# preshanth/rfi_toolbox

Measured on AMD Instinct MI355X. Metric: training patches/sec (128x128x3), higher is better.
Workload: dtype f32; 1 GPU; UNet(3,1,32) train step (fwd+BCE/dice+bwd+clip+Adam), batch 64/GPU x 128x128x3 NHWC, BASELINE configs[1] shape on the reference's U-Net (the '3-layer CNN' of configs[1] is not in the reference; its builder-defined form runs with --workload cnn3); global_batch=64, parallelism=dp1, params=7765985

## Files before the change

rfi_toolbox_amd/csrc/api.cpp:

```cpp
#include <dlfcn.h>

#include <algorithm>
#include <cmath>

#include "model.hpp"

using namespace rfi;

namespace rfi {
static thread_local std::string g_last_error;
void set_last_error(const std::string& msg) { g_last_error = msg; }
}

void rfi_ctx::activate() const { RFI_CHECK_HIP(hipSetDevice(device)); }

void* rfi_ctx::alloc(size_t bytes) {
    void* p = nullptr;
    if (bytes == 0) bytes = 16;
    RFI_CHECK_HIP(hipMalloc(&p, bytes));
    allocs[p] = bytes;
    return p;
}
void rfi_ctx::release(void* p) {
    if (!p) return;
// ... 432 lines not shown
int rfi_model_set_head_sigmoid(rfi_model* m, int enabled) {
    return guarded([&] {
        RFI_REQUIRE(plain_unet(m), "set_head_sigmoid: U-Net models only");
        m->head_sigmoid = enabled != 0;
    });
}

namespace {

void copy_on_stream(rfi_ctx* ctx, void* dst, const void* src, size_t bytes, hipMemcpyKind kind) {
    if (kind == hipMemcpyDeviceToDevice) launch_copy_d2d(ctx, dst, src, bytes);
    else RFI_CHECK_HIP(hipMemcpyAsync(dst, src, bytes, kind, ctx->stream));
}
const float* stage_input(rfi_model* m, const float* x, int x_mem, int n, int h, int w, bool nchw) {
    const size_t cnt = (size_t)n * h * w * m->in_ch;
    const float* dev = x;
    if (x_mem == RFI_HOST) {
        float* st = m->buf(nchw ? m->x_stage2 : m->x_stage);
        RFI_CHECK_HIP(hipMemcpyAsync(st, x, cnt * sizeof(float), hipMemcpyHostToDevice, m->ctx->stream));
        dev = st;
    }
    if (nchw) {
        launch_nchw_to_nhwc(m->ctx, dev, n, m->in_ch, h, w, m->buf(m->x_stage));
        dev = m->buf(m->x_stage);
    }
    return dev;
}
const uint8_t* stage_labels(rfi_model* m, const uint8_t* y, int y_mem, int n, int h, int w) {
    if (y_mem == RFI_DEVICE) return y;
    uint8_t* st = reinterpret_cast<uint8_t*>(m->buf(m->lab_stage));
    RFI_CHECK_HIP(hipMemcpyAsync(st, y, (size_t)n * h * w * m->out_scale * m->out_scale, hipMemcpyHostToDevice, m->ctx->stream));
    return st;
}
void sync_if_host(rfi_model* m, int mem_a, int mem_b = RFI_DEVICE) {
    static const bool always = getenv("RFI_SYNC_ALWAYS") != nullptr;
    if (always || mem_a != RFI_DEVICE || mem_b != RFI_DEVICE) RFI_CHECK_HIP(hipStreamSynchronize(m->ctx->stream));
}
void emit_logits(rfi_model* m, float* out, int out_mem, int n, int h, int w, bool nchw) {
    h *= m->out_scale; w *= m->out_scale;
    const size_t cnt = (size_t)n * h * w * m->out_ch;
    const float* src = m->buf(m->head_sigmoid ? m->probs : m->logits);
    if (nchw && m->out_ch > 1) {
        launch_nhwc_to_nchw(m->ctx, src, n, m->out_ch, h, w, m->buf(m->out_stage));
        src = m->buf(m->out_stage);
    }
    copy_on_stream(m->ctx, out, src, cnt * sizeof(float), out_mem == RFI_DEVICE ? hipMemcpyDeviceToDevice : hipMemcpyDeviceToHost);
    sync_if_host(m, out_mem);
}
float read_scalar(rfi_model* m, const float* dev) {
    RFI_CHECK_HIP(hipMemcpyAsync(m->ctx->pinned, dev, sizeof(float), hipMemcpyDeviceToHost, m->ctx->stream));
    RFI_CHECK_HIP(hipStreamSynchronize(m->ctx->stream));
    return m->ctx->pinned[0];
}
void check_hyper(const rfi_hyper* hp) {
    RFI_REQUIRE(hp, "null hyper-parameters");
    RFI_REQUIRE(hp->lr >= 0 && hp->eps >= 0 && hp->weight_decay >= 0, "Adam: lr, eps, weight_decay must be >= 0");
    RFI_REQUIRE(hp->beta1 >= 0 && hp->beta1 < 1 && hp->beta2 >= 0 && hp->beta2 < 1, "Adam: betas must be in [0,1)");
}


void backward_with_exchange(rfi_model* m, const float* x, const uint8_t* y, int n, int h, int w) {
    struct Flag { rfi_model* m; ~Flag() { m->exchange_in_backward = false; } } flag{m};
    m->exchange_in_backward = true;
    m->backward(x, y, n, h, w);
}
void exchange_and_apply(rfi_model* m, const rfi_hyper& hp) {
    if (m->ctx->exchange_active()) {
        m->exchange_join();
        m->apply(hp, 1.0f / (float)m->ctx->exchange_world());
    } else {
        m->apply(hp, 1.0f);
    }
}

}

int rfi_model_forward_nhwc(rfi_model* m, const float* x, int x_mem, int n, int h, int w, float* logits,
                           int logits_mem) {
    return guarded([&] {
        m->ctx->activate();
        m->prepare(n, h, w);
        const float* xd = stage_input(m, x, x_mem, n, h, w, false);
        m->forward(xd, n, h, w, m->training);
        emit_logits(m, logits, logits_mem, n, h, w, false);
    });
}
int rfi_model_forward_nchw(rfi_model* m, const float* x, int x_mem, int n, int h, int w, float* logits,
                           int logits_mem) {
    return guarded([&] {
        m->ctx->activate();
        m->prepare(n, h, w);
        const float* xd = stage_input(m, x, x_mem, n, h, w, true);
        m->forward(xd, n, h, w, m->training);
        emit_logits(m, logits, logits_mem, n, h, w, true);
    });
}

int rfi_train_forward_backward(rfi_model* m, const float* x, int x_mem, const uint8_t* labels,
                               int labels_mem, int n, int h, int w, float* loss_out) {
    return guarded([&] {
        m->ctx->activate();
        m->prepare(n, h, w);
        const float* xd = stage_input(m, x, x_mem, n, h, w, false);
        const uint8_t* yd = stage_labels(m, labels, labels_mem, n, h, w);
        m->forward(xd, n, h, w, true);
        m->loss_forward(yd, n, h, w);
        m->backward(xd, yd, n, h, w);
        if (loss_out) *loss_out = m->last_loss = read_scalar(m, m->d_scalars);
    });
}
int rfi_train_apply(rfi_model* m, const rfi_hyper* hp, float grad_scale, float* grad_norm_out) {
    return guarded([&] {
        check_hyper(hp);
        m->ctx->activate();
        RFI_REQUIRE(m->pN > 0, "rfi_train_apply: no gradients (call rfi_train_forward_backward first)");
        m->apply(*hp, grad_scale);
        if (grad_norm_out) *grad_norm_out = m->last_norm = read_scalar(m, m->d_scalars + 1);
    });
}
int rfi_train_step(rfi_model* m, const float* x, int x_mem, const uint8_t* labels, int labels_mem,
                   int n, int h, int w, const rfi_hyper* hp, float* loss_out) {
    return guarded([&] {
        check_hyper(hp);
        m->ctx->activate();
        m->prepare(n, h, w);
        const float* xd = stage_input(m, x, x_mem, n, h, w, false);
        const uint8_t* yd = stage_labels(m, labels, labels_mem, n, h, w);
        m->forward(xd, n, h, w, true);
        m->loss_forward(yd, n, h, w);
        backward_with_exchange(m, xd, yd, n, h, w);
        exchange_and_apply(m, *hp);
        RFI_CHECK_HIP(hipMemcpyAsync(m->ctx->pinned, m->d_scalars, 2 * sizeof(float), hipMemcpyDeviceToHost,
                                     m->ctx->stream));
        RFI_CHECK_HIP(hipStreamSynchronize(m->ctx->stream));
        m->last_loss = m->ctx->pinned[0];
        m->last_norm = m->ctx->pinned[1];
        if (loss_out) *loss_out = m->last_loss;
    });
}
int rfi_train_step_async(rfi_model* m, const float* x_dev, const uint8_t* labels_dev, int n, int h,
                         int w, const rfi_hyper* hp) {
    return guarded([&] {
        check_hyper(hp);
        m->ctx->activate();
        m->prepare(n, h, w);
        m->forward(x_dev, n, h, w, true);
        m->loss_forward(labels_dev, n, h, w);
        backward_with_exchange(m, x_dev, labels_dev, n, h, w);
        exchange_and_apply(m, *hp);
    });
}
int rfi_model_backward_dlogits(rfi_model* m, const float* x, int x_mem, const float* dlogits, int dlogits_mem, int n, int h,
                               int w) {
    return guarded([&] {
        RFI_REQUIRE(m->gx >= 0, "backward_dlogits: mask / RPN / box heads only");
        RFI_REQUIRE(m->pN == n && m->pH == h && m->pW == w, "backward_dlogits: run the forward pass on this input first");
        m->ctx->activate();
        const float* xd = stage_input(m, x, x_mem, n, h, w, false);
        const size_t cnt = (size_t)n * h * w * m->out_scale * m->out_scale * m->out_ch;
        copy_on_stream(m->ctx, m->buf(m->dlogits), dlogits, cnt * sizeof(float),
                       dlogits_mem == RFI_DEVICE ? hipMemcpyDeviceToDevice : hipMemcpyHostToDevice);
        struct Flag { rfi_model* m; ~Flag() { m->ext_dlogits = false; } } flag{m};
        m->ext_dlogits = true;
        m->backward(xd, nullptr, n, h, w);
        sync_if_host(m, x_mem, dlogits_mem);
    });
}
int rfi_backbone_forward(rfi_model* m, const float* x, int x_mem, int n, int h, int w, float* const feats[5], int feats_mem) {
    return guarded([&] {
        auto* b = dynamic_cast<BackboneModel*>(m);
        RFI_REQUIRE(b && feats, "backbone_forward: ResNet-50-FPN models only");
        m->ctx->activate();
        m->prepare(n, h, w);
        const float* xd = stage_input(m, x, x_mem, n, h, w, false);
        m->forward(xd, n, h, w, false);
        for (int i = 0; i < 5; ++i) {
            if (!feats[i]) continue;
            const int lvl = i + 2;
            const size_t cnt = (size_t)n * (h >> lvl) * (w >> lvl) * m->out_ch;
            copy_on_stream(m->ctx, feats[i], m->buf(i < 4 ? b->fP[i] : b->fP6), cnt * sizeof(float),
                           feats_mem == RFI_DEVICE ? hipMemcpyDeviceToDevice : hipMemcpyDeviceToHost);
        }
        sync_if_host(m, x_mem, feats_mem);
    });
}
int rfi_backbone_backward(rfi_model* m, const float* x, int x_mem, int n, int h, int w, const float* const dfeats[5], int dfeats_mem) {
    return guarded([&] {
        auto* b = dynamic_cast<BackboneModel*>(m);
        RFI_REQUIRE(b && dfeats, "backbone_backward: ResNet-50-FPN models only");
        RFI_REQUIRE(m->pN == n && m->pH == h && m->pW == w, "backbone_backward: run the forward pass on this input first");
        m->ctx->activate();
        const float* xd = stage_input(m, x, x_mem, n, h, w, false);
        for (int i = 0; i < 5; ++i) {
            const int lvl = i + 2;
            const size_t cnt = (size_t)n * (h >> lvl) * (w >> lvl) * m->out_ch;
            float* dst = m->buf(i < 4 ? b->fdP[i] : b->fdP6);
            if (dfeats[i])
                copy_on_stream(m->ctx, dst, dfeats[i], cnt * sizeof(float),
// ... 757 lines not shown
```

rfi_toolbox_amd/csrc/conv_stem.hip:

```cpp
#include <algorithm>

#include "ws_common.hpp"

namespace rfi {
namespace {

using namespace ws;

struct StemDev {
    const float* x;
    int N, H, W;
    const float* w;
    const float* bias;
    float* y;
    int y_ps, Cout;
    double* stats;
};

constexpr int TH = 8, TW = 32, HH = TH + 2, HW = TW + 2, HP = HH * HW;
constexpr int PLANE = HP * 8;

template <int NT>
__global__ __launch_bounds__(256) void conv_stem_kernel(StemDev d) {
    __shared__ __attribute__((aligned(16))) unsigned char s_img[3 * PLANE];
    __shared__ double s_stat[4 * NT * 64 * 2];
    const int tid = threadIdx.x, lane = tid & 63, wave = tid >> 6;
    const int li = lane & 31, kh = lane >> 5;

    bf16x8 bfr[NT][3][3];
#pragma unroll
    for (int nt = 0; nt < NT; ++nt)
#pragma unroll
        for (int s = 0; s < 3; ++s) {
            f32x4 v[2];
#pragma unroll
            for (int h = 0; h < 2; ++h) {
                const int tap = 4 * s + 2 * kh + h, co = nt * 32 + li;
                v[h] = f32x4{0.f, 0.f, 0.f, 0.f};
                if (tap < 9 && co < d.Cout) v[h] = *reinterpret_cast<const f32x4*>(d.w + ((size_t)tap * d.Cout + co) * 4);
            }
            unsigned pl[3][4];
            split_pair(v[0].x, v[0].y, pl[0][0], pl[1][0], pl[2][0]);
            split_pair(v[0].z, v[0].w, pl[0][1], pl[1][1], pl[2][1]);
            split_pair(v[1].x, v[1].y, pl[0][2], pl[1][2], pl[2][2]);
            split_pair(v[1].z, v[1].w, pl[0][3], pl[1][3], pl[2][3]);
#pragma unroll
            for (int p = 0; p < 3; ++p) bfr[nt][s][p] = __builtin_bit_cast(bf16x8, u32x4{pl[p][0], pl[p][1], pl[p][2], pl[p][3]});
        }
    int toff[3][2];
#pragma unroll
    for (int s = 0; s < 3; ++s)
#pragma unroll
        for (int h = 0; h < 2; ++h) {
            const int tap = std::min(4 * s + 2 * kh + h, 8);
            toff[s][h] = ((tap / 3) * HW + tap % 3 + li) * 8;
        }
    float bias[NT];
#pragma unroll
    for (int nt = 0; nt < NT; ++nt) bias[nt] = (d.bias && nt * 32 + li < d.Cout) ? d.bias[nt * 32 + li] : 0.0f;
    double d1[NT], d2[NT];
#pragma unroll
    for (int nt = 0; nt < NT; ++nt) d1[nt] = d2[nt] = 0.0;

    const int tiles_x = (d.W + TW - 1) / TW, tiles_y = (d.H + TH - 1) / TH;
    const int ntiles = d.N * tiles_y * tiles_x;
    for (int t = blockIdx.x; t < ntiles; t += gridDim.x) {
        const int ox0 = (t % tiles_x) * TW, oy0 = ((t / tiles_x) % tiles_y) * TH, n = t / (tiles_x * tiles_y);
        __syncthreads();
        for (int idx = tid; idx < HP; idx += 256) {
            const int iy = oy0 - 1 + idx / HW, ix = ox0 - 1 + idx % HW;
            f32x4 v = {0.f, 0.f, 0.f, 0.f};
            if ((unsigned)iy < (unsigned)d.H && (unsigned)ix < (unsigned)d.W)
                v = *reinterpret_cast<const f32x4*>(d.x + ((size_t)(n * d.H + iy) * d.W + ix) * 4);
            unsigned h0, m0, l0, h1, m1, l1;
            split_pair(v.x, v.y, h0, m0, l0);
            split_pair(v.z, v.w, h1, m1, l1);
            *reinterpret_cast<u32x2*>(s_img + idx * 8) = u32x2{h0, h1};
            *reinterpret_cast<u32x2*>(s_img + PLANE + idx * 8) = u32x2{m0, m1};
            *reinterpret_cast<u32x2*>(s_img + 2 * PLANE + idx * 8) = u32x2{l0, l1};
        }
        __syncthreads();
#pragma unroll
        for (int rb = 0; rb < 2; ++rb) {
            const int row = 2 * wave + rb;
            const unsigned char* base = s_img + row * HW * 8;
            f32x16 acc[NT];
#pragma unroll
            for (int nt = 0; nt < NT; ++nt)
#pragma unroll
                for (int r = 0; r < 16; ++r) acc[nt][r] = 0.0f;
#pragma unroll
            for (int s = 0; s < 3; ++s) {
                bf16x8 af[3];
#pragma unroll
                for (int p = 0; p < 3; ++p) {
                    const u32x2 a0 = *reinterpret_cast<const u32x2*>(base + p * PLANE + toff[s][0]);
                    const u32x2 a1 = *reinterpret_cast<const u32x2*>(base + p * PLANE + toff[s][1]);
                    af[p] = __builtin_bit_cast(bf16x8, u32x4{a0.x, a0.y, a1.x, a1.y});
                }
#pragma unroll
                for (int nt = 0; nt < NT; ++nt) acc[nt] = mma3(af, bfr[nt][s], acc[nt]);
            }
            const int oy = oy0 + row;
#pragma unroll
            for (int nt = 0; nt < NT; ++nt) {
                const int co = nt * 32 + li;
                float s1 = 0.0f, s2 = 0.0f;
#pragma unroll
                for (int r = 0; r < 16; ++r) {
                    const int ox = ox0 + (r & 3) + 8 * (r >> 2) + 4 * kh;
                    const float v = acc[nt][r] + bias[nt];
                    if (oy < d.H && ox < d.W && co < d.Cout) {
                        d.y[((size_t)(n * d.H + oy) * d.W + ox) * d.y_ps + co] = v;
                        s1 += v;
                        s2 += v * v;
                    }
                }
                d1[nt] += (double)s1;
                d2[nt] += (double)s2;
            }
        }
    }
    if (d.stats) {
#pragma unroll
        for (int nt = 0; nt < NT; ++nt) {
            s_stat[((wave * NT + nt) * 64 + lane) * 2] = d1[nt];
            s_stat[((wave * NT + nt) * 64 + lane) * 2 + 1] = d2[nt];
        }
        __syncthreads();
        if (tid < 32 * NT && tid < d.Cout) {
            const int nt = tid >> 5, cl = tid & 31;
            double t1 = 0.0, t2 = 0.0;
#pragma unroll
            for (int w = 0; w < 4; ++w)
#pragma unroll
                for (int h = 0; h < 2; ++h) {
                    t1 += s_stat[((w * NT + nt) * 64 + h * 32 + cl) * 2];
                    t2 += s_stat[((w * NT + nt) * 64 + h * 32 + cl) * 2 + 1];
                }
            d.stats[((size_t)blockIdx.x * d.Cout + tid) * 2] = t1;
            d.stats[((size_t)blockIdx.x * d.Cout + tid) * 2 + 1] = t2;
        }
    }
}

}

bool conv_stem_eligible(const ConvArgs& a) {
    if (!(a.R == 3 && a.S == 1 && a.pad == 1 && a.zgroups == 1 && a.Cin == 4 && a.x.pstride == 4 && (a.Cout == 32 || a.Cout == 64))) return false;
    if (a.Hin != a.H || a.Win != a.W || a.Hout != a.H || a.Wout != a.W || a.osy != 1 || a.osx != 1 || a.ooy || a.oox) return false;
    if (a.xf.scale || a.fold || a.y16) return false;
    if ((reinterpret_cast<uintptr_t>(a.x.p) | reinterpret_cast<uintptr_t>(a.w)) & 15) return false;
    return (int64_t)a.N * a.H * a.W * std::max<int64_t>(a.y.pstride, 4) * 4 < ((int64_t)1 << 40);
}

void launch_conv_stem(rfi_ctx* ctx, ConvArgs& a) {
    RFI_REQUIRE(conv_stem_eligible(a) && a.bf16x3, "conv_stem: shape or arithmetic not eligible");
    const int ntiles = a.N * (int)cdiv(a.H, TH) * (int)cdiv(a.W, TW);
    int GX = std::min(ntiles, 1024);
    if (a.stats && GX > a.stats_max_records) GX = a.stats_max_records > 0 ? a.stats_max_records : GX;
    if (a.stats && a.stats_max_records > 0) a.stats_records = GX;
    else { a.stats = nullptr; a.stats_records = 0; }
    StemDev d{a.x.p, a.N, a.H, a.W, a.w, a.bias, a.y.p, (int)a.y.pstride, a.Cout, a.stats};
    const double flops = a.algo_flops >= 0 ? a.algo_flops : 2.0 * a.N * a.H * a.W * 9.0 * 3 * a.Cout;
    const double bytes = 4.0 * ((double)a.N * a.H * a.W * (4 + a.Cout) + 9.0 * 4 * a.Cout);
    std::string label;
    if (ctx->profiling)
        label = "conv_stem N" + std::to_string(a.N) + " " + std::to_string(a.H) + "x" + std::to_string(a.W) + " 4->" + std::to_string(a.Cout) +
                " 3xbf16";
    ProfScope ps(ctx, FAM_CONV_MFMA, flops, bytes, label);
    if (a.Cout == 32) hipLaunchKernelGGL(conv_stem_kernel<1>, dim3(GX), dim3(256), 0, ctx->stream, d);
    else hipLaunchKernelGGL(conv_stem_kernel<2>, dim3(GX), dim3(256), 0, ctx->stream, d);
    check_launch("conv_stem");
}

}
```

rfi_toolbox_amd/csrc/elem_kernels.hip:

```cpp
#include <hip/hip_ext.h>

#include "kernels.hpp"

namespace rfi {

namespace {

constexpr int kBlock = 256;
constexpr int kFinCh = 2;
constexpr int kFinLanes = kBlock / kFinCh;

__device__ __forceinline__ double wave_sum(double v) {
#pragma unroll
    for (int o = 32; o > 0; o >>= 1) v += __shfl_down(v, o, 64);
    return v;
}

__device__ __forceinline__ double finish_sum(double v, double* red) {
#pragma unroll
    for (int o = 32; o >= kFinCh; o >>= 1) v += __shfl_xor(v, o, 64);
    const int wave = threadIdx.x >> 6, lane = threadIdx.x & 63;
    __syncthreads();
    if (lane < kFinCh) red[wave * kFinCh + lane] = v;
    __syncthreads();
// ... 71 lines not shown
        v[e] = (float)h;
    }
    *reinterpret_cast<uint2*>(p) = make_uint2((unsigned)q[0] | ((unsigned)q[1] << 16), (unsigned)q[2] | ((unsigned)q[3] << 16));
}
template <int V, int NQ>
__device__ __forceinline__ void row_lane_reduce(double (&acc)[NQ][V], double* red, int CL, int RL, int cl,
                                                int rl) {
#pragma unroll
    for (int q = 0; q < NQ; ++q)
#pragma unroll
        for (int v = 0; v < V; ++v) red[(q * V + v) * kBlock + threadIdx.x] = acc[q][v];
    __syncthreads();
    const int NF = RL >= 4 ? 4 : 1;
    if (rl < NF) {
#pragma unroll
        for (int q = 0; q < NQ; ++q)
#pragma unroll
            for (int v = 0; v < V; ++v) {
                double t0 = rl == 0 ? acc[q][v] : 0.0, t1 = 0.0;
                const double* rp = red + (q * V + v) * kBlock + cl;
                int k = rl == 0 ? NF : rl;
                for (; k + NF < RL; k += 2 * NF) {
                    t0 += rp[k * CL];
                    t1 += rp[(k + NF) * CL];
                }
                if (k < RL) t0 += rp[k * CL];
                acc[q][v] = t0 + t1;
            }
    }
    if (NF > 1) {
        __syncthreads();
        if (rl > 0 && rl < NF) {
#pragma unroll
            for (int q = 0; q < NQ; ++q)
#pragma unroll
                for (int v = 0; v < V; ++v) red[(q * V + v) * kBlock + threadIdx.x] = acc[q][v];
        }
        __syncthreads();
        if (rl == 0) {
#pragma unroll
            for (int q = 0; q < NQ; ++q)
#pragma unroll
                for (int v = 0; v < V; ++v) {
                    double t = acc[q][v];
                    for (int j = 1; j < NF; ++j) t += red[(q * V + v) * kBlock + j * CL + cl];
                    acc[q][v] = t;
                }
        }
    }
}

__device__ __forceinline__ float act_f(float a, float slope) { return a > 0.0f ? a : (slope != 0.0f ? a * slope : 0.0f); }
__device__ __forceinline__ float dact_f(float z, float g, float slope) { return z > 0.0f ? g : g * slope; }

template <int V>
__global__ void bn_stats_kernel(const float* __restrict__ y, int64_t M, int C, int CL,
                                int64_t rows_per_block, double* __restrict__ partial) {
    __shared__ double red[2 * V * kBlock];
    const int RL = kBlock / CL;
    const int cl = threadIdx.x % CL, rl = threadIdx.x / CL;
    const int c = (blockIdx.y * CL + cl) * V;
    const int64_t r0 = (int64_t)blockIdx.x * rows_per_block;
    int64_t r1 = r0 + rows_per_block;
    if (r1 > M) r1 = M;
    double acc[2][V];
#pragma unroll
    for (int v = 0; v < V; ++v) acc[0][v] = acc[1][v] = 0;
    if (c < C) {
        for (int64_t r = r0 + rl; r < r1; r += RL) {
            float x[V];
            ldv<V>(y + r * C + c, x);
#pragma unroll
            for (int v = 0; v < V; ++v) {
                const double d = (double)x[v];
                acc[0][v] += d;
                acc[1][v] += d * d;
            }
        }
    }
    row_lane_reduce<V, 2>(acc, red, CL, RL, cl, rl);
    if (rl == 0 && c < C) {
#pragma unroll
        for (int v = 0; v < V; ++v) {
            partial[((int64_t)blockIdx.x * C + c + v) * 2 + 0] = acc[0][v];
            partial[((int64_t)blockIdx.x * C + c + v) * 2 + 1] = acc[1][v];
        }
    }
}

__global__ void bn_finalize_kernel(const double* __restrict__ partial, int records, int C,
                                   double count, const float* __restrict__ gamma,
                                   const float* __restrict__ beta, float* __restrict__ running_mean,
                                   float* __restrict__ running_var, int ema_repeats,
                                   float* __restrict__ mean_out, float* __restrict__ invstd_out,
                                   float* __restrict__ scale, float* __restrict__ shift,
                                   float* __restrict__ var_out) {
    __shared__ double red[2 * kBlock];
    const int cl = threadIdx.x & (kFinCh - 1), rl = threadIdx.x / kFinCh;
    const int c = blockIdx.x * kFinCh + cl;
    double s1 = 0, s2 = 0;
    if (c < C) {
        for (int r = rl; r < records; r += kFinLanes) {
            s1 += partial[((int64_t)r * C + c) * 2 + 0];
            s2 += partial[((int64_t)r * C + c) * 2 + 1];
        }
    }
// ... 197 lines not shown
                        o[v] = g[v] * (dz - k1[v] - xh * k2[v]);
                        if (SUMS) p1[v] += o[v];
                    }
                    *reinterpret_cast<uint4*>(planes + r * pl_stride + c) =
                        make_uint4(pack_bf16x2(o[0], o[1]), pack_bf16x2(o[2], o[3]), pack_bf16x2(o[4], o[5]), pack_bf16x2(o[6], o[7]));
                }
            }
            if (SUMS) {
#pragma unroll
                for (int v = 0; v < 8; ++v) acc[0][v] += (double)p1[v];
            }
        }
    }
    if constexpr (SUMS) {
        row_lane_reduce<8, 1>(acc, red, CL, RL, cl, rl);
        if (rl == 0 && c < C) {
#pragma unroll
            for (int v = 0; v < 8; ++v) partial[(int64_t)blockIdx.x * C + c + v] = acc[0][v];
        }
    }
}

__global__ void bn_bwd_finalize_kernel(const double* __restrict__ partial, int records, int C,
                                       double count, float* c1, float* c2, float* dgamma,
                                       float* dbeta) {
    __shared__ double red[2 * kBlock];
    const int cl = threadIdx.x & (kFinCh - 1), rl = threadIdx.x / kFinCh;
    const int c = blockIdx.x * kFinCh + cl;
    double s1 = 0, s2 = 0;
    if (c < C) {
        for (int r = rl; r < records; r += kFinLanes) {
            s1 += partial[((int64_t)r * C + c) * 2 + 0];
            s2 += partial[((int64_t)r * C + c) * 2 + 1];
        }
    }
    s1 = finish_sum(s1, red);
    s2 = finish_sum(s2, red);
    if (rl == 0 && c < C) {
        c1[c] = (float)(s1 / count);
        c2[c] = (float)(s2 / count);
        dgamma[c] = (float)s2;
        dbeta[c] = (float)s1;
    }
}

template <int V>
__global__ void bn_bwd_apply_kernel(void* __restrict__ da_, int da16, const void* __restrict__ y, int y16, int64_t yps, int64_t M,
                                    int C, int CL, int64_t rows_per_block,
                                    const float* __restrict__ scale, const float* __restrict__ shift,
                                    const float* __restrict__ mean, const float* __restrict__ invstd,
                                    const float* __restrict__ gamma, const float* __restrict__ c1,
                                    const float* __restrict__ c2, double* __restrict__ partial, float slope,
                                    unsigned short* __restrict__ planes, int64_t pl_stride, int P,
                                    const float* __restrict__ head_dl, const float* __restrict__ head_w) {
    __shared__ double red[V * kBlock];
    const int RL = kBlock / CL;
    const int cl = threadIdx.x % CL, rl = threadIdx.x / CL;
    const int c = (blockIdx.y * CL + cl) * V;
    const int64_t r0 = (int64_t)blockIdx.x * rows_per_block;
    int64_t r1 = r0 + rows_per_block;
    if (r1 > M) r1 = M;
    double acc[1][V];
#pragma unroll
    for (int v = 0; v < V; ++v) acc[0][v] = 0;
    if (c < C) {
        float sc[V], sh[V], mu[V], is[V], g[V], k1[V], k2[V];
        ldv<V>(scale + c, sc); ldv<V>(shift + c, sh); ldv<V>(mean + c, mu); ldv<V>(invstd + c, is);
        ldv<V>(gamma + c, g); ldv<V>(c1 + c, k1); ldv<V>(c2 + c, k2);
#pragma unroll
        for (int v = 0; v < V; ++v) g[v] = g[v] * is[v];
        float hw[V];
#pragma unroll
        for (int v = 0; v < V; ++v) hw[v] = head_dl ? head_w[c + v] : 0.0f;
        constexpr int U = 4;
        for (int64_t rb = r0 + rl; rb < r1; rb += (int64_t)U * RL) {
          float yu[U][V], du[U][V];
#pragma unroll
          for (int k = 0; k < U; ++k) {
              const int64_t r = rb + (int64_t)k * RL;
              if (r < r1) {
                  ldy<V>(y, y16, r * yps + c, yu[k]);
                  if (head_dl) {
                      const float d = head_dl[r];
#pragma unroll
                      for (int v = 0; v < V; ++v) du[k][v] = d * hw[v];
                  } else {
                      ldy<V>(da_, da16, r * C + c, du[k]);
                  }
              }
          }
#pragma unroll
          for (int k = 0; k < U; ++k) {
            const int64_t r = rb + (int64_t)k * RL;
            if (r >= r1) break;
            float yv[V], dv[V], o[V];
#pragma unroll
            for (int v = 0; v < V; ++v) { yv[v] = yu[k][v]; dv[v] = du[k][v]; }
#pragma unroll
            for (int v = 0; v < V; ++v) {
                const float dz = dact_f(yv[v] * sc[v] + sh[v], dv[v], slope);
                const float xh = (yv[v] - mu[v]) * is[v];
                o[v] = g[v] * (dz - k1[v] - xh * k2[v]);
                acc[0][v] += (double)o[v];
            }
            if (planes) {
                unsigned short* q = planes + r * pl_stride + (int64_t)(c >> 4) * (P * 16) + (c & 15);
                float res[V];
#pragma unroll
                for (int v = 0; v < V; ++v) res[v] = o[v];
                for (int p = 0; p < P; ++p) {
                    unsigned short hq[V];
#pragma unroll
                    for (int v = 0; v < V; ++v) {
                        const __bf16 h = (__bf16)res[v];
                        hq[v] = __builtin_bit_cast(unsigned short, h);
                        res[v] -= (float)h;
                    }
                    if constexpr (V == 4)
                        *reinterpret_cast<uint2*>(q + p * 16) = make_uint2((unsigned)hq[0] | ((unsigned)hq[1] << 16), (unsigned)hq[2] | ((unsigned)hq[3] << 16));
                    else
                        q[p * 16] = hq[0];
                }
            } else {
                stv<V>(static_cast<float*>(da_) + r * C + c, o);
            }
          }
        }
    }
    row_lane_reduce<V, 1>(acc, red, CL, RL, cl, rl);
    if (rl == 0 && c < C) {
#pragma unroll
        for (int v = 0; v < V; ++v) partial[(int64_t)blockIdx.x * C + c + v] = acc[0][v];
    }
}

__global__ void finish_channel_sum_kernel(const double* __restrict__ partial, int records,
// ... 236 lines not shown
         i += (int64_t)gridDim.x * blockDim.x) {
        const int c = (int)(i % C);
        const int64_t pix = i / C;
        const int x = (int)(pix % W);
        const int yy = (int)((pix / W) % H);
        if (yy >= He || x >= We) da[pix * C + c] = dskip[pix * dskip_ps + c];
    }
}

__global__ void head_fwd_kernel(const float* __restrict__ y, int64_t M, int C,
                                const float* __restrict__ scale, const float* __restrict__ shift,
                                const float* __restrict__ w, const float* __restrict__ b, int Cout,
                                float* __restrict__ logits, float slope) {
    const int lane16 = threadIdx.x & 15;
    const int64_t m = ((int64_t)blockIdx.x * blockDim.x + threadIdx.x) >> 4;
    if (m >= M) return;
    for (int o = 0; o < Cout; ++o) {
        float acc = 0.0f;
        for (int c = lane16; c < C; c += 16) {
            float a = y[m * C + c] * scale[c] + shift[c];
            a = act_f(a, slope);
            acc += a * w[o * C + c];
        }
#pragma unroll
        for (int off = 8; off > 0; off >>= 1) acc += __shfl_down(acc, off, 16);
        if (lane16 == 0) logits[m * Cout + o] = acc + b[o];
    }
}

template <int L>
__global__ __launch_bounds__(256) void head_fwd_vec_kernel(const void* __restrict__ y, int y16, int64_t yps, int64_t M, int C,
                                                           const float* __restrict__ scale, const float* __restrict__ shift,
                                                           const float* __restrict__ w, const float* __restrict__ b, int Cout,
                                                           float* __restrict__ logits, float slope) {
    const int lane = threadIdx.x & (L - 1);
    const int64_t m = ((int64_t)blockIdx.x * blockDim.x + threadIdx.x) / L;
    if (m >= M) return;
    const int C4 = C >> 2;
    for (int o = 0; o < Cout; ++o) {
        float acc = 0.0f;
        for (int c4 = lane; c4 < C4; c4 += L) {
            float yv[4], sc[4], sh[4], wv[4];
            ldy<4>(y, y16, m * yps + 4 * c4, yv); ldv<4>(scale + 4 * c4, sc); ldv<4>(shift + 4 * c4, sh);
            ldv<4>(w + (int64_t)o * C + 4 * c4, wv);
#pragma unroll
            for (int v = 0; v < 4; ++v) acc += act_f(yv[v] * sc[v] + sh[v], slope) * wv[v];
        }
#pragma unroll
        for (int off = L / 2; off > 0; off >>= 1) acc += __shfl_down(acc, off, L);
        if (lane == 0) logits[m * Cout + o] = acc + b[o];
    }
}

__device__ __forceinline__ float sigmoidf_(float x) { return 1.0f / (1.0f + expf(-x)); }

__global__ void loss_reduce_kernel(const float* __restrict__ logits, const uint8_t* __restrict__ labels,
                                   int64_t count, double* __restrict__ partial) {
    __shared__ double red[4][kBlock / 64];
    double s[4] = {0, 0, 0, 0};
    for (int64_t i = (int64_t)blockIdx.x * blockDim.x + threadIdx.x; i < count;
         i += (int64_t)gridDim.x * blockDim.x) {
        const float x = logits[i];
        const float t = labels[i] ? 1.0f : 0.0f;
        const float bce = fmaxf(x, 0.0f) - x * t + log1pf(expf(-fabsf(x)));
        const float p = sigmoidf_(x);
        s[0] += (double)bce;
        s[1] += (double)(p * t);
        s[2] += (double)p;
        s[3] += (double)t;
    }
    const int wave = threadIdx.x >> 6, lane = threadIdx.x & 63;
#pragma unroll
    for (int k = 0; k < 4; ++k) {
        double v = wave_sum(s[k]);
        if (lane == 0) red[k][wave] = v;
    }
    __syncthreads();
    if (threadIdx.x < 4) {
        double v = 0;
        for (int wv = 0; wv < kBlock / 64; ++wv) v += red[threadIdx.x][wv];
        partial[(int64_t)blockIdx.x * 4 + threadIdx.x] = v;
    }
}

__global__ void loss_finish_kernel(const double* __restrict__ partial, int blocks, double count,
                                   double* __restrict__ sums4, float* __restrict__ loss_out) {
    __shared__ double red[4][kBlock / 64];
    double s[4] = {0, 0, 0, 0};
    for (int b = threadIdx.x; b < blocks; b += blockDim.x)
        for (int k = 0; k < 4; ++k) s[k] += partial[(int64_t)b * 4 + k];
    const int wave = threadIdx.x >> 6, lane = threadIdx.x & 63;
#pragma unroll
    for (int k = 0; k < 4; ++k) {
        double v = wave_sum(s[k]);
        if (lane == 0) red[k][wave] = v;
    }
    __syncthreads();
    if (threadIdx.x == 0) {
        double t[4];
        for (int k = 0; k < 4; ++k) {
            t[k] = 0;
            for (int wv = 0; wv < kBlock / 64; ++wv) t[k] += red[k][wv];
            sums4[k] = t[k];
        }
        const float bce = (float)(t[0] / count);
        const float inter = (float)t[1], sp = (float)t[2], st = (float)t[3];
        const float dice = 1.0f - (2.0f * inter + 1.0f) / (sp + st + 1.0f);
        loss_out[0] = bce + dice;
    }
}

__global__ void loss_bwd_kernel(const float* __restrict__ logits, const uint8_t* __restrict__ labels,
                                int64_t count, const double* __restrict__ sums4,
                                float* __restrict__ dlogits) {
    const float inter = (float)sums4[1], sp = (float)sums4[2], st = (float)sums4[3];
    const float D = sp + st + 1.0f;
    const float num = 2.0f * inter + 1.0f;
    const float invD2 = 1.0f / (D * D);
    const float invN = (float)(1.0 / (double)count);
    for (int64_t i = (int64_t)blockIdx.x * blockDim.x + threadIdx.x; i < count;
         i += (int64_t)gridDim.x * blockDim.x) {
        const float x = logits[i];
        const float t = labels[i] ? 1.0f : 0.0f;
        const float p = sigmoidf_(x);
        const float ddice = -(2.0f * t * D - num) * invD2;
        dlogits[i] = (p - t) * invN + ddice * p * (1.0f - p);
    }
}

__device__ __forceinline__ float focal_elem(float x, float t, float alpha, float gamma) {
    const float p = sigmoidf_(x);
    const float ce = fmaxf(x, 0.0f) - x * t + log1pf(expf(-fabsf(x)));
    const float pt = p * t + (1.0f - p) * (1.0f - t);
    const float at = alpha >= 0.0f ? alpha * t + (1.0f - alpha) * (1.0f - t) : 1.0f;
    return at * powf(1.0f - pt, gamma) * ce;
}
__global__ void focal_reduce_kernel(const float* __restrict__ logits, const uint8_t* __restrict__ labels,
                                    int64_t count, float alpha, float gamma, double* __restrict__ partial) {
    __shared__ double red[kBlock / 64];
    double s = 0;
    for (int64_t i = (int64_t)blockIdx.x * blockDim.x + threadIdx.x; i < count; i += (int64_t)gridDim.x * blockDim.x)
        s += (double)focal_elem(logits[i], labels[i] ? 1.0f : 0.0f, alpha, gamma);
    s = wave_sum(s);
    if ((threadIdx.x & 63) == 0) red[threadIdx.x >> 6] = s;
    __syncthreads();
    if (threadIdx.x == 0) {
        double t = 0;
        for (int k = 0; k < kBlock / 64; ++k) t += red[k];
        partial[blockIdx.x] = t;
    }
}
__global__ void focal_finish_kernel(const double* __restrict__ partial, int blocks, double count,
                                    float* __restrict__ loss_out) {
    __shared__ double red[kBlock / 64];
    double s = 0;
    for (int b = threadIdx.x; b < blocks; b += blockDim.x) s += partial[b];
    s = wave_sum(s);
    if ((threadIdx.x & 63) == 0) red[threadIdx.x >> 6] = s;
    __syncthreads();
    if (threadIdx.x == 0) {
        double t = 0;
        for (int k = 0; k < kBlock / 64; ++k) t += red[k];
        loss_out[0] = (float)(t / count);
    }
}
__global__ void focal_bwd_kernel(const float* __restrict__ logits, const uint8_t* __restrict__ labels, int64_t count,
                                 float alpha, float gamma, float* __restrict__ dlogits) {
    const float invN = (float)(1.0 / (double)count);
    for (int64_t i = (int64_t)blockIdx.x * blockDim.x + threadIdx.x; i < count; i += (int64_t)gridDim.x * blockDim.x) {
        const float x = logits[i];
        const bool pos = labels[i] != 0;
        const float p = sigmoidf_(x);
        const float sp_neg = fmaxf(-x, 0.0f) + log1pf(expf(-fabsf(x)));
        const float sp_pos = fmaxf(x, 0.0f) + log1pf(expf(-fabsf(x)));
        float g;
        if (pos) {
            const float a = alpha >= 0.0f ? alpha : 1.0f;
            g = a * powf(1.0f - p, gamma) * (gamma * p * (-sp_neg) - (1.0f - p));
        } else {
            const float a = alpha >= 0.0f ? 1.0f - alpha : 1.0f;
// ... 116 lines not shown
                if (bn_records) {
#pragma unroll
                    for (int v = 0; v < 4; ++v) {
                        const float dz = dact_f(yv[v] * sc[v] + sh[v], g[v], slope);
                        const float xh = (yv[v] - mu[v]) * is[v];
                        q1[v] += (double)dz;
                        q2[v] += (double)dz * (double)xh;
                    }
                }
                sb += (double)d;
              }
            }
        }
#pragma unroll
        for (int v = 0; v < 4; ++v) red[v * kBlock + threadIdx.x] = sw[v];
        __syncthreads();
        if (rl == 0 && c < C) {
#pragma unroll
            for (int v = 0; v < 4; ++v) {
                double t = sw[v];
                for (int k = 1; k < RL; ++k) t += red[v * kBlock + k * CL + cl];
                partial[(int64_t)blockIdx.x * pstride + (int64_t)o * C + c + v] = t;
            }
        }
        __syncthreads();
        if (blockIdx.y == 0 && cl == 0) red[rl] = sb;
        __syncthreads();
        if (blockIdx.y == 0 && threadIdx.x == 0) {
            double t = 0;
            for (int k = 0; k < RL; ++k) t += red[k];
            partial[(int64_t)blockIdx.x * pstride + (int64_t)Cout * C + o] = t;
        }
        __syncthreads();
    }
    if (bn_records) {
#pragma unroll
        for (int q = 0; q < 2; ++q) {
#pragma unroll
            for (int v = 0; v < 4; ++v) red[v * kBlock + threadIdx.x] = q == 0 ? q1[v] : q2[v];
            __syncthreads();
            if (rl == 0 && c < C) {
#pragma unroll
                for (int v = 0; v < 4; ++v) {
                    double t = q == 0 ? q1[v] : q2[v];
                    for (int k = 1; k < RL; ++k) t += red[v * kBlock + k * CL + cl];
                    bn_records[((int64_t)blockIdx.x * C + c + v) * 2 + q] = t;
                }
            }
            __syncthreads();
        }
    }
}

__global__ void nchw_to_nhwc_kernel(const float* __restrict__ src, int N, int C, int H, int W,
                                    float* __restrict__ dst) {
    const int64_t total = (int64_t)N * C * H * W;
    for (int64_t i = (int64_t)blockIdx.x * blockDim.x + threadIdx.x; i < total;
         i += (int64_t)gridDim.x * blockDim.x) {
        const int c = (int)(i % C);
        int64_t t = i / C;
        const int x = (int)(t % W);
        t /= W;
        const int yy = (int)(t % H);
        const int n = (int)(t / H);
        dst[i] = src[(((int64_t)n * C + c) * H + yy) * W + x];
    }
}
__global__ void nhwc_to_nchw_kernel(const float* __restrict__ src, int N, int C, int H, int W,
                                    float* __restrict__ dst) {
    const int64_t total = (int64_t)N * C * H * W;
    for (int64_t i = (int64_t)blockIdx.x * blockDim.x + threadIdx.x; i < total;
         i += (int64_t)gridDim.x * blockDim.x) {
        const int x = (int)(i % W);
        int64_t t = i / W;
        const int yy = (int)(t % H);
        t /= H;
        const int c = (int)(t % C);
        const int n = (int)(t / C);
        dst[i] = src[(((int64_t)n * H + yy) * W + x) * C + c];
    }
}
__global__ void weight_to_dgrad_kernel(const float* __restrict__ wf, int taps, int Cout, int Cin,
                                       int flip, float* __restrict__ wd) {
    const int64_t total = (int64_t)taps * Cout * Cin;
    for (int64_t i = (int64_t)blockIdx.x * blockDim.x + threadIdx.x; i < total;
         i += (int64_t)gridDim.x * blockDim.x) {
        const int co = (int)(i % Cout);
        int64_t t = i / Cout;
        const int ci = (int)(t % Cin);
        const int tp = (int)(t / Cin);
        const int ts = flip ? (taps - 1 - tp) : tp;
        wd[i] = wf[((int64_t)ts * Cout + co) * Cin + ci];
    }
}
__global__ __launch_bounds__(256) void weight_to_dgrad_batched_kernel(const RelayoutDesc* __restrict__ descs, int n,
                                                                     const float* __restrict__ src, float* __restrict__ dst) {
    __shared__ float tile[32][33];
    const int64_t b = blockIdx.x;
    int l = 0;
    while (l + 1 < n && descs[l + 1].tile0 <= b) ++l;
    const RelayoutDesc d = descs[l];
    const float* __restrict__ wf = src + d.src_off;
    float* __restrict__ wd = dst + d.dst_off;
    const int tci = (d.cin + 31) / 32, tco = (d.cout + 31) / 32;
    const int t = (int)(b - d.tile0);
    const int tp = t / (tci * tco), r = t % (tci * tco);
// ... 12 lines not shown
        if (co < d.cout && ci < d.cin) wd[((int64_t)tp * d.cin + ci) * d.cout + co] = tile[tx][ty + 8 * k];
    }
}
__global__ void relu_bwd_kernel(float4* __restrict__ dA, const float4* __restrict__ Y, int64_t n4) {
    for (int64_t i = (int64_t)blockIdx.x * blockDim.x + threadIdx.x; i < n4;
         i += (int64_t)gridDim.x * blockDim.x) {
        float4 g = dA[i];
        const float4 y = Y[i];
        g.x = y.x > 0.0f ? g.x : 0.0f;
        g.y = y.y > 0.0f ? g.y : 0.0f;
        g.z = y.z > 0.0f ? g.z : 0.0f;
        g.w = y.w > 0.0f ? g.w : 0.0f;
        dA[i] = g;
    }
}
__global__ void pad_channels_kernel(const float* __restrict__ s, int64_t M, int c, int cp,
                                    float* __restrict__ d) {
    const int64_t total = M * cp;
    for (int64_t i = (int64_t)blockIdx.x * blockDim.x + threadIdx.x; i < total;
         i += (int64_t)gridDim.x * blockDim.x) {
        const int k = (int)(i % cp);
        d[i] = k < c ? s[(i / cp) * c + k] : 0.0f;
    }
}
__global__ void u8_to_f32_kernel(const uint8_t* __restrict__ s, int64_t n, float* __restrict__ d) {
    for (int64_t i = (int64_t)blockIdx.x * blockDim.x + threadIdx.x; i < n;
         i += (int64_t)gridDim.x * blockDim.x)
        d[i] = (float)s[i];
}

__global__ void sumsq_kernel(const float* __restrict__ g, int64_t n, double* __restrict__ partial) {
    __shared__ double red[kBlock / 64];
    double s = 0;
    const int64_t n4 = n >> 2;
    const float4* g4 = reinterpret_cast<const float4*>(g);
    for (int64_t i = (int64_t)blockIdx.x * blockDim.x + threadIdx.x; i < n4;
         i += (int64_t)gridDim.x * blockDim.x) {
        const float4 v = g4[i];
        s += (double)v.x * v.x + (double)v.y * v.y + (double)v.z * v.z + (double)v.w * v.w;
    }
    if (blockIdx.x == 0 && threadIdx.x < (n & 3)) {
        const float v = g[(n4 << 2) + threadIdx.x];
        s += (double)v * v;
    }
    s = wave_sum(s);
    if ((threadIdx.x & 63) == 0) red[threadIdx.x >> 6] = s;
    __syncthreads();
    if (threadIdx.x == 0) {
        double t = 0;
        for (int k = 0; k < kBlock / 64; ++k) t += red[k];
        partial[blockIdx.x] = t;
    }
}
__global__ void sumsq_finish_kernel(const double* __restrict__ partial, int blocks,
                                    double* __restrict__ out) {
    __shared__ double red[kBlock / 64];
    double s = 0;
    for (int b = threadIdx.x; b < blocks; b += blockDim.x) s += partial[b];
    s = wave_sum(s);
    if ((threadIdx.x & 63) == 0) red[threadIdx.x >> 6] = s;
    __syncthreads();
    if (threadIdx.x == 0) {
        double t = 0;
        for (int k = 0; k < kBlock / 64; ++k) t += red[k];
        out[0] = t;
    }
}

__global__ void adam_kernel(AdamArgs a) {
    const float norm = (float)sqrt(a.sumsq[0]) * a.grad_scale;
    float coef = a.max_norm / (norm + 1e-6f);
    coef = coef > 1.0f ? 1.0f : coef;
    if (a.max_norm <= 0.0f) coef = 1.0f;
    const float gs = a.grad_scale;
    for (int64_t i = (int64_t)blockIdx.x * blockDim.x + threadIdx.x; i < a.n;
         i += (int64_t)gridDim.x * blockDim.x) {
        const float p = a.p[i];
        float g = (a.g[i] * gs) * coef;
        g = __fmaf_rn(a.wd, p, g);
        const float m0 = a.m[i];
        const float m = __fmaf_rn(a.one_minus_beta1, g - m0, m0);
        const float v = __fmaf_rn(a.one_minus_beta2 * g, g, a.beta2 * a.v[i]);
        a.m[i] = m;
        a.v[i] = v;
        const float denom = sqrtf(v) / a.bc2_sqrt + a.eps;
        a.p[i] = p + (a.neg_step * m) / denom;
    }
    if (blockIdx.x == 0 && threadIdx.x == 0 && a.norm_out) a.norm_out[0] = norm;
}

__global__ void scale_inplace_kernel(float* __restrict__ x, int64_t n, float f) {
    for (int64_t i = (int64_t)blockIdx.x * blockDim.x + threadIdx.x; i < n; i += (int64_t)gridDim.x * blockDim.x) x[i] *= f;
}
__global__ void reduce_slabs_kernel(const float* __restrict__ slabs, int nslabs, int group, int kstride,
                                    int64_t n, float* __restrict__ out, int64_t out_rowstride) {
    const int base = blockIdx.y * group;
    int cnt = nslabs - base;
    if (cnt > group) cnt = group;
    for (int64_t i = (int64_t)blockIdx.x * blockDim.x + threadIdx.x; i < n;
         i += (int64_t)gridDim.x * blockDim.x) {
        float s = 0.0f;
        for (int k = 0; k < cnt; ++k) s += slabs[((int64_t)base + (int64_t)k) * kstride * n + i];
        out[(int64_t)blockIdx.y * out_rowstride * n + i] = s;
    }
}

__global__ __launch_bounds__(256) void reduce_slabs_vec4_kernel(const float* __restrict__ slabs, int nslabs, int group, int kstride,
                                                               int64_t n4, float* __restrict__ out, int64_t out_rowstride) {
    typedef float f32x4 __attribute__((ext_vector_type(4)));
    const int base = blockIdx.y * group;
    int cnt = nslabs - base;
    if (cnt > group) cnt = group;
    const f32x4* __restrict__ src = reinterpret_cast<const f32x4*>(slabs) + (int64_t)base * kstride * n4;
    f32x4* __restrict__ dst = reinterpret_cast<f32x4*>(out) + (int64_t)blockIdx.y * out_rowstride * n4;
    const int64_t step = (int64_t)kstride * n4;
    for (int64_t i = (int64_t)blockIdx.x * blockDim.x + threadIdx.x; i < n4; i += (int64_t)gridDim.x * blockDim.x) {
        f32x4 s = {0.f, 0.f, 0.f, 0.f};
        int k = 0;
        for (; k + 8 <= cnt; k += 8) {
            f32x4 v[8];
#pragma unroll
            for (int u = 0; u < 8; ++u) v[u] = __builtin_nontemporal_load(src + (int64_t)(k + u) * step + i);
#pragma unroll
// ... 59 lines not shown
    return (size_t)kMaxRowBlocks * C * 2 * 2;
}

void launch_bn_bwd_finalize_records(rfi_ctx* ctx, const float* partial_ws, int records, int64_t M, int C, float* c1,
                                    float* c2, float* dgamma, float* dbeta) {
    ProfScope ps(ctx, FAM_BN);
    hipLaunchKernelGGL(bn_bwd_finalize_kernel, dim3((int)cdiv(C, kFinCh)), dim3(kBlock), 0, ctx->stream,
                       reinterpret_cast<const double*>(partial_ws), records, C, (double)M, c1, c2, dgamma, dbeta);
    check_launch("bn_bwd_finalize");
}

void launch_bn_bwd_reduce(rfi_ctx* ctx, YRef da, YRef y, int64_t M, int C,
                          const float* scale, const float* shift, const float* mean,
                          const float* invstd, float* partial_ws, float* c1, float* c2,
                          float* dgamma, float* dbeta, float slope) {
    ChanGeom g = geom_rows(M, C);
    const bool fast16 = da.bf16 && y.bf16 && C % 8 == 0 && da.stride(C) == C && y.stride(C) % 8 == 0 &&
                        !((reinterpret_cast<uintptr_t>(da.p) | reinterpret_cast<uintptr_t>(y.p) | reinterpret_cast<uintptr_t>(scale) |
                           reinterpret_cast<uintptr_t>(shift) | reinterpret_cast<uintptr_t>(mean) | reinterpret_cast<uintptr_t>(invstd)) & 15);
    if (fast16) {
        g = chan_geom(M, C, kMaxRowBlocks, true, 8);
        ProfScope ps(ctx, FAM_BN, 0, (double)M * C * 4);
        hipLaunchKernelGGL(bn_bwd_reduce16_kernel, dim3(g.rblocks, g.cblocks), dim3(kBlock), 0, ctx->stream,
                           static_cast<const unsigned short*>(da.p), static_cast<const unsigned short*>(y.p), y.stride(C), M, C, g.CL,
                           g.rows_per_block, scale, shift, mean, invstd, reinterpret_cast<double*>(partial_ws), slope);
        check_launch("bn_bwd_reduce16");
    } else {
        RFI_REQUIRE(da.stride(C) == C && (!da.bf16 || g.V == 4), "bn_bwd_reduce: the gradient tensor must be dense (bfloat16: C % 4 == 0)");
        ProfScope ps(ctx, FAM_BN, 0, (double)M * C * ((y.bf16 ? 2 : 4) + (da.bf16 ? 2 : 4)));
        if (g.V == 4)
            hipLaunchKernelGGL(bn_bwd_reduce_kernel<4>, dim3(g.rblocks, g.cblocks), dim3(kBlock), 0,
                               ctx->stream, da.p, da.bf16, y.p, y.bf16, y.stride(C), M, C, g.CL, g.rows_per_block, scale, shift, mean, invstd,
                               reinterpret_cast<double*>(partial_ws), slope);
        else
            hipLaunchKernelGGL(bn_bwd_reduce_kernel<1>, dim3(g.rblocks, g.cblocks), dim3(kBlock), 0,
                               ctx->stream, da.p, da.bf16, y.p, y.bf16, y.stride(C), M, C, g.CL, g.rows_per_block, scale, shift, mean, invstd,
                               reinterpret_cast<double*>(partial_ws), slope);
        check_launch("bn_bwd_reduce");
    }
    {
        ProfScope ps(ctx, FAM_BN);
        hipLaunchKernelGGL(bn_bwd_finalize_kernel, dim3((int)cdiv(C, kFinCh)), dim3(kBlock), 0, ctx->stream,
                           reinterpret_cast<const double*>(partial_ws), g.rblocks, C, (double)M, c1, c2,
                           dgamma, dbeta);
        check_launch("bn_bwd_finalize");
    }
}

void launch_bn_bwd_apply(rfi_ctx* ctx, YRef da_inout, YRef y, int64_t M, int C,
                         const float* scale, const float* shift, const float* mean,
                         const float* invstd, const float* gamma, const float* c1, const float* c2,
                         float* partial_ws, float* dbias, float slope, unsigned short* planes_out,
                         int64_t planes_pstride, int planes_P, hipEvent_t done, bool finish_dbias, const float* head_dl,
                         const float* head_w) {
    ChanGeom g = geom_rows(M, C);
    const bool fast16 = da_inout.bf16 && y.bf16 && planes_out && planes_P == 1 && !head_dl && C % 8 == 0 && da_inout.stride(C) == C &&
                        y.stride(C) % 8 == 0 && planes_pstride % 8 == 0 &&
                        !((reinterpret_cast<uintptr_t>(da_inout.p) | reinterpret_cast<uintptr_t>(y.p) | reinterpret_cast<uintptr_t>(planes_out) |
                           reinterpret_cast<uintptr_t>(scale) | reinterpret_cast<uintptr_t>(shift) | reinterpret_cast<uintptr_t>(mean) |
                           reinterpret_cast<uintptr_t>(invstd) | reinterpret_cast<uintptr_t>(gamma) | reinterpret_cast<uintptr_t>(c1) |
                           reinterpret_cast<uintptr_t>(c2)) & 15);
    if (fast16) {
        const ChanGeom g4 = g;
        g = chan_geom(M, C, kMaxRowBlocks, true, 8);
        if (dbias) {
            g.rows_per_block = g4.rows_per_block;
            g.rblocks = g4.rblocks;
        }
        {
            ProfScope ps(ctx, FAM_BN, 0, (double)M * C * 6);
            auto launch = [&](auto kernel) {
                hipExtLaunchKernelGGL(kernel, dim3(g.rblocks, g.cblocks), dim3(kBlock), 0, ctx->stream, nullptr, done, 0,
                                      static_cast<const unsigned short*>(da_inout.p), static_cast<const unsigned short*>(y.p), y.stride(C), M, C, g.CL,
                                      g.rows_per_block, scale, shift, mean, invstd, gamma, c1, c2, reinterpret_cast<double*>(partial_ws), slope,
                                      planes_out, planes_pstride);
            };
            if (dbias) launch(bn_bwd_apply16_kernel<true>);
            else launch(bn_bwd_apply16_kernel<false>);
            check_launch("bn_bwd_apply16");
        }
        if (dbias && finish_dbias) {
            ProfScope ps(ctx, FAM_BN);
            hipLaunchKernelGGL(finish_channel_sum_kernel, dim3((int)cdiv(C, kFinCh)), dim3(kBlock), 0, ctx->stream,
                               reinterpret_cast<const double*>(partial_ws), g.rblocks, (int64_t)C, C, dbias);
            check_launch("finish_channel_sum");
        }
        return;
    }
    {
        RFI_REQUIRE(da_inout.stride(C) == C && (!da_inout.bf16 || (planes_out && g.V == 4)),
                    "bn_bwd_apply: a bfloat16 gradient tensor needs the plane output and C % 4 == 0");
        ProfScope ps(ctx, FAM_BN, 0, (double)M * C * ((planes_out ? 8 + 2 * planes_P : 12) - (y.bf16 ? 2 : 0) - (da_inout.bf16 ? 2 : 0)));
        auto launch = [&](auto kernel) {
            hipExtLaunchKernelGGL(kernel, dim3(g.rblocks, g.cblocks), dim3(kBlock), 0, ctx->stream, nullptr, done, 0,
                                  const_cast<void*>(da_inout.p), da_inout.bf16, y.p, y.bf16, y.stride(C), M, C, g.CL, g.rows_per_block, scale, shift, mean, invstd, gamma,
                                  c1, c2, reinterpret_cast<double*>(partial_ws), slope, planes_out, planes_pstride, planes_P, head_dl, head_w);
        };
        if (g.V == 4) launch(bn_bwd_apply_kernel<4>);
        else launch(bn_bwd_apply_kernel<1>);
        check_launch("bn_bwd_apply");
    }
    if (dbias && finish_dbias) launch_bn_bwd_apply_finish(ctx, partial_ws, M, C, dbias);
}
void launch_bn_bwd_apply_finish(rfi_ctx* ctx, const float* partial_ws, int64_t M, int C, float* dbias) {
    ChanGeom g = geom_rows(M, C);
    ProfScope ps(ctx, FAM_BN);
    hipLaunchKernelGGL(finish_channel_sum_kernel, dim3((int)cdiv(C, kFinCh)), dim3(kBlock), 0,
                       ctx->stream, reinterpret_cast<const double*>(partial_ws), g.rblocks, (int64_t)C, C, dbias);
    check_launch("finish_channel_sum");
}

int bn_bwd_apply_records(int64_t M, int C) { return geom_rows(M, C).rblocks; }
void launch_finish_channel_sums_batched(rfi_ctx* ctx, const FinishSumDesc* descs_dev, int n, int max_count) {
    if (n <= 0) return;
    ProfScope ps(ctx, FAM_BN);
    hipLaunchKernelGGL(finish_channel_sum_batched_kernel, dim3((int)cdiv(max_count, kFinCh), n), dim3(kBlock), 0, ctx->stream, descs_dev);
    check_launch("finish_channel_sum_batched");
}

size_t channel_sum_ws_floats(int64_t M, int C) {
    (void)M;
    return (size_t)kMaxRowBlocks * C * 2;
}
void launch_channel_sum(rfi_ctx* ctx, YRef v, int64_t M, int C, float* partial_ws, float* out, bool finish) {
    ChanGeom g = geom_rows(M, C);
    const int pstride = (int)v.stride(C);
    const bool vec = g.V == 4 && pstride % 4 == 0 && (reinterpret_cast<uintptr_t>(v.p) & (v.bf16 ? 7 : 15)) == 0;
    RFI_REQUIRE(finish || vec, "channel_sum: deferred finishing needs the vector path (C % 4 == 0, an aligned view)");
    RFI_REQUIRE(vec || !v.bf16, "channel_sum: a bfloat16 view needs C % 4 == 0 and 8-byte aligned rows");
    if (!vec && g.V == 4) g = geom_rows(M, C, false);
    {
        ProfScope ps(ctx, FAM_REDUCE, 0, (double)M * C * (v.bf16 ? 2 : 4));
        if (g.V == 4)
            hipLaunchKernelGGL(channel_sum_kernel<4>, dim3(g.rblocks, g.cblocks), dim3(kBlock), 0, ctx->stream,
                               v.p, v.bf16, pstride, M, C, g.CL, g.rows_per_block,
                               reinterpret_cast<double*>(partial_ws));
        else
            hipLaunchKernelGGL(channel_sum_kernel<1>, dim3(g.rblocks, g.cblocks), dim3(kBlock), 0, ctx->stream,
                           v.p, v.bf16, pstride, M, C, g.CL, g.rows_per_block,
                           reinterpret_cast<double*>(partial_ws));
        check_launch("channel_sum");
    }
    if (finish) {
        ProfScope ps(ctx, FAM_REDUCE);
        hipLaunchKernelGGL(finish_channel_sum_kernel, dim3((int)cdiv(C, kFinCh)), dim3(kBlock), 0,
                           ctx->stream, reinterpret_cast<const double*>(partial_ws), g.rblocks, (int64_t)C, C, out);
        check_launch("finish_channel_sum");
    }
}
// ... 122 lines not shown
    }
    {
        ProfScope ps(ctx, FAM_ELEMWISE);
        hipLaunchKernelGGL(loss_finish_kernel, dim3(1), dim3(kBlock), 0, ctx->stream, partial_ws, blocks,
                           (double)count, sums4, loss_out);
        check_launch("loss_finish");
    }
}
void launch_focal_reduce(rfi_ctx* ctx, const float* logits, const uint8_t* labels, int64_t count, float alpha,
                         float gamma, double* partial_ws, float* loss_out) {
    int blocks = grid_for(count, 1024);
    {
        ProfScope ps(ctx, FAM_ELEMWISE, 0, (double)count * 5);
        hipLaunchKernelGGL(focal_reduce_kernel, dim3(blocks), dim3(kBlock), 0, ctx->stream, logits, labels, count,
                           alpha, gamma, partial_ws);
        check_launch("focal_reduce");
    }
    {
        ProfScope ps(ctx, FAM_ELEMWISE);
        hipLaunchKernelGGL(focal_finish_kernel, dim3(1), dim3(kBlock), 0, ctx->stream, partial_ws, blocks,
                           (double)count, loss_out);
        check_launch("focal_finish");
    }
}
void launch_focal_bwd(rfi_ctx* ctx, const float* logits, const uint8_t* labels, int64_t count, float alpha,
                      float gamma, float* dlogits) {
    ProfScope ps(ctx, FAM_ELEMWISE, 0, (double)count * 9);
    hipLaunchKernelGGL(focal_bwd_kernel, dim3(grid_for(count)), dim3(kBlock), 0, ctx->stream, logits, labels,
                       count, alpha, gamma, dlogits);
    check_launch("focal_bwd");
}
void launch_loss_bwd(rfi_ctx* ctx, const float* logits, const uint8_t* labels, int64_t count,
                     const double* sums4, float* dlogits) {
    ProfScope ps(ctx, FAM_ELEMWISE, 0, (double)count * 9);
    hipLaunchKernelGGL(loss_bwd_kernel, dim3(grid_for(count)), dim3(kBlock), 0, ctx->stream, logits,
                       labels, count, sums4, dlogits);
    check_launch("loss_bwd");
}

void launch_sigmoid_fwd(rfi_ctx* ctx, const float* z, int64_t n, float* x) {
    ProfScope ps(ctx, FAM_ELEMWISE, 0, (double)n * 8);
    hipLaunchKernelGGL(sigmoid_fwd_kernel, dim3(grid_for(n)), dim3(kBlock), 0, ctx->stream, z, n, x);
    check_launch("sigmoid_fwd");
}
void launch_sigmoid_bwd(rfi_ctx* ctx, const float* x, int64_t n, float* d_inout) {
    ProfScope ps(ctx, FAM_ELEMWISE, 0, (double)n * 12);
    hipLaunchKernelGGL(sigmoid_bwd_kernel, dim3(grid_for(n)), dim3(kBlock), 0, ctx->stream, x, n, d_inout);
    check_launch("sigmoid_bwd");
}

size_t head_bwd_ws_floats(int64_t M, int C, int Cout) {
    (void)M;
    return (size_t)kMaxRowBlocks * ((size_t)Cout * C + Cout) * 2;
}
int launch_head_bwd(rfi_ctx* ctx, YRef yr, int64_t M, int C, const float* scale,
                    const float* shift, const float* w, int Cout, const float* dlogits, float* da,
                    float* partial_ws, float* dw, float* db, float slope, const float* bn_mean, const float* bn_invstd,
                    float* bn_records_ws, unsigned short* da16, bool* skip_da, bool finish) {
    const bool may_skip = skip_da && *skip_da;
    if (skip_da) *skip_da = false;
    int bn_records = 0;
    const bool vec = C % 4 == 0 && !((reinterpret_cast<uintptr_t>(yr.p) | reinterpret_cast<uintptr_t>(da) |
                                      reinterpret_cast<uintptr_t>(scale) | reinterpret_cast<uintptr_t>(shift) |
                                      reinterpret_cast<uintptr_t>(w)) & 15) && yr.stride(C) % 4 == 0;
    RFI_REQUIRE(vec || !yr.bf16, "head_bwd: a bfloat16 input needs C % 4 == 0");
    RFI_REQUIRE(finish || vec, "head_bwd: deferred finishing needs the vector path (C % 4 == 0, 16-byte aligned tensors)");
    RFI_REQUIRE(!da16 || (vec && Cout == 1 && !(reinterpret_cast<uintptr_t>(da16) & 7)), "head_bwd: a bfloat16 gradient tensor needs C % 4 == 0 and one output channel");
    const float* y = static_cast<const float*>(yr.p);
    ChanGeom g = geom_rows(M, C, vec);
    {
        ProfScope ps(ctx, FAM_ELEMWISE, 4.0 * M * C * Cout, (double)M * C * (yr.bf16 ? 6 : 8));
        if (vec) {
            const bool sums = bn_records_ws && bn_mean && bn_invstd && Cout == 1 &&
                              !((reinterpret_cast<uintptr_t>(bn_mean) | reinterpret_cast<uintptr_t>(bn_invstd)) & 15);
            hipLaunchKernelGGL(head_bwd_vec_kernel, dim3(g.rblocks, g.cblocks), dim3(kBlock), 0, ctx->stream, yr.p, yr.bf16,
                               yr.stride(C), M, C, g.CL, g.rows_per_block, scale, shift, w, Cout, dlogits, da,
                               reinterpret_cast<double*>(partial_ws), slope, bn_mean, bn_invstd,
                               sums ? reinterpret_cast<double*>(bn_records_ws) : nullptr, da16, (sums && may_skip && !da16) ? 0 : 1);
            if (sums) bn_records = g.rblocks;
            if (sums && may_skip && !da16) *skip_da = true;
        }
        else
            hipLaunchKernelGGL(head_bwd_kernel, dim3(g.rblocks, g.cblocks), dim3(kBlock), 0, ctx->stream, y,
                               M, C, g.CL, g.rows_per_block, scale, shift, w, Cout, dlogits, da,
                               reinterpret_cast<double*>(partial_ws), slope);
        check_launch("head_bwd");
    }
    if (finish) {
        const int n = Cout * C + Cout;
        ProfScope ps(ctx, FAM_REDUCE);
        hipLaunchKernelGGL(finish_channel_sum_kernel, dim3((int)cdiv(Cout * C, kFinCh)), dim3(kBlock), 0,
                           ctx->stream, reinterpret_cast<const double*>(partial_ws), g.rblocks, (int64_t)n, Cout * C, dw);
        check_launch("head_bwd_finish_dw");
    }
    if (finish) {
        const int n = Cout * C + Cout;
        ProfScope ps(ctx, FAM_REDUCE);
        hipLaunchKernelGGL(finish_channel_sum_kernel, dim3((int)cdiv(Cout, kFinCh)), dim3(kBlock), 0,
                           ctx->stream, reinterpret_cast<const double*>(partial_ws) + (size_t)Cout * C,
                           g.rblocks, (int64_t)n, Cout, db);
        check_launch("head_bwd_finish_db");
    }
    return bn_records;
}

void launch_nchw_to_nhwc(rfi_ctx* ctx, const float* src, int N, int C, int H, int W, float* dst) {
// ... 7 lines not shown
    const int64_t total = (int64_t)N * C * H * W;
    ProfScope ps(ctx, FAM_ELEMWISE, 0, (double)total * 8);
    hipLaunchKernelGGL(nhwc_to_nchw_kernel, dim3(grid_for(total)), dim3(kBlock), 0, ctx->stream, src, N,
                       C, H, W, dst);
    check_launch("nhwc_to_nchw");
}
void launch_weight_to_dgrad(rfi_ctx* ctx, const float* wf, int taps, int Cout, int Cin, int flip,
                            float* wd) {
    const int64_t total = (int64_t)taps * Cout * Cin;
    ProfScope ps(ctx, FAM_ELEMWISE, 0, (double)total * 8);
    hipLaunchKernelGGL(weight_to_dgrad_kernel, dim3(grid_for(total)), dim3(kBlock), 0, ctx->stream, wf,
                       taps, Cout, Cin, flip, wd);
    check_launch("weight_to_dgrad");
}
int64_t relayout_assign_tiles(RelayoutDesc* descs, int n) {
    int64_t t = 0;
    for (int i = 0; i < n; ++i) {
        descs[i].tile0 = t;
        t += (int64_t)descs[i].taps * ((descs[i].cout + 31) / 32) * ((descs[i].cin + 31) / 32);
    }
    return t;
}
void launch_weight_to_dgrad_batched(rfi_ctx* ctx, const RelayoutDesc* descs_dev, int n, const float* src,
                                    float* dst, double total_bytes, int64_t total_tiles) {
    RFI_REQUIRE(total_tiles > 0 && total_tiles < ((int64_t)1 << 31), "weight_to_dgrad_batched: bad tile count");
    ProfScope ps(ctx, FAM_ELEMWISE, 0, total_bytes);
    hipLaunchKernelGGL(weight_to_dgrad_batched_kernel, dim3((unsigned)total_tiles), dim3(256), 0, ctx->stream, descs_dev, n,
                       src, dst);
    check_launch("weight_to_dgrad_batched");
}
void launch_relu_bwd(rfi_ctx* ctx, float* dA, const float* Y, int64_t n) {
    RFI_REQUIRE(n % 4 == 0, "relu_bwd: element count must be a multiple of 4");
    ProfScope ps(ctx, FAM_ELEMWISE, 0, (double)n * 12);
    hipLaunchKernelGGL(relu_bwd_kernel, dim3(grid_for(n / 4)), dim3(kBlock), 0, ctx->stream,
                       reinterpret_cast<float4*>(dA), reinterpret_cast<const float4*>(Y), n / 4);
    check_launch("relu_bwd");
}
void launch_pad_channels(rfi_ctx* ctx, const float* src, int64_t M, int c, int cp, float* dst) {
    ProfScope ps(ctx, FAM_ELEMWISE, 0, (double)M * (c + cp) * 4);
    hipLaunchKernelGGL(pad_channels_kernel, dim3(grid_for(M * cp)), dim3(kBlock), 0, ctx->stream, src, M, c,
                       cp, dst);
    check_launch("pad_channels");
}
void launch_u8_to_f32(rfi_ctx* ctx, const uint8_t* src, int64_t n, float* dst) {
    ProfScope ps(ctx, FAM_ELEMWISE, 0, (double)n * 5);
    hipLaunchKernelGGL(u8_to_f32_kernel, dim3(grid_for(n)), dim3(kBlock), 0, ctx->stream, src, n, dst);
    check_launch("u8_to_f32");
}

size_t sumsq_ws_doubles(int64_t n) {
    (void)n;
    return 1024 + 8;
}
void launch_sumsq(rfi_ctx* ctx, const float* g, int64_t n, double* partial_ws, double* sumsq) {
    int blocks = grid_for(n / 4 + 1, 1024);
    {
        ProfScope ps(ctx, FAM_OPTIM, 0, (double)n * 4);
        hipLaunchKernelGGL(sumsq_kernel, dim3(blocks), dim3(kBlock), 0, ctx->stream, g, n, partial_ws);
        check_launch("sumsq");
    }
    {
        ProfScope ps(ctx, FAM_OPTIM);
        hipLaunchKernelGGL(sumsq_finish_kernel, dim3(1), dim3(kBlock), 0, ctx->stream, partial_ws, blocks,
                           sumsq);
        check_launch("sumsq_finish");
    }
}
void launch_adam(rfi_ctx* ctx, const AdamArgs& a) {
    ProfScope ps(ctx, FAM_OPTIM, 0, (double)a.n * 28);
    hipLaunchKernelGGL(adam_kernel, dim3(grid_for(a.n)), dim3(kBlock), 0, ctx->stream, a);
    check_launch("adam");
}

void launch_scale_inplace(rfi_ctx* ctx, float* x, int64_t n, float f) {
    if (n <= 0) return;
    ProfScope ps(ctx, FAM_COMM, 0, (double)n * 8);
    hipLaunchKernelGGL(scale_inplace_kernel, dim3(grid_for(n)), dim3(kBlock), 0, ctx->stream, x, n, f);
    check_launch("scale_inplace");
}
void launch_reduce_slabs(rfi_ctx* ctx, const float* slabs, int nslabs, int64_t n, float* out) {
    float* s = const_cast<float*>(slabs);
    int count = nslabs;
    int stride = 1;
    const bool vec = n % 4 == 0 && !((reinterpret_cast<uintptr_t>(slabs) | reinterpret_cast<uintptr_t>(out)) & 15);
    while (count > 32) {
        const int groups = (int)cdiv(count, 32);
        ProfScope ps(ctx, FAM_REDUCE, 0, (double)n * 4 * (count + groups));
        if (vec)
            hipLaunchKernelGGL(reduce_slabs_vec4_kernel, dim3(grid_for(n / 4, 1024), groups), dim3(kBlock), 0, ctx->stream, s, count, 32,
                               stride, n / 4, s, (int64_t)32 * stride);
        else
        hipLaunchKernelGGL(reduce_slabs_kernel, dim3(grid_for(n, 1024), groups), dim3(kBlock), 0,
                           ctx->stream, s, count, 32, stride, n, s, (int64_t)32 * stride);
        check_launch("reduce_slabs_fold");
        count = groups;
        stride *= 32;
    }
    ProfScope ps(ctx, FAM_REDUCE, 0, (double)n * 4 * (count + 1));
    if (vec)
        hipLaunchKernelGGL(reduce_slabs_vec4_kernel, dim3(grid_for(n / 4, 1024), 1), dim3(kBlock), 0, ctx->stream, s, count, 32, stride,
                           n / 4, out, (int64_t)0);
    else
    hipLaunchKernelGGL(reduce_slabs_kernel, dim3(grid_for(n, 1024), 1), dim3(kBlock), 0, ctx->stream, s,
                       count, 32, stride, n, out, (int64_t)0);
    check_launch("reduce_slabs");
}

}
```

rfi_toolbox_amd/csrc/kernels.hpp:

```cpp
#pragma once
#include "common.hpp"

namespace rfi {

struct InXform {
    const float* scale = nullptr;
    const float* shift = nullptr;
    int relu = 0;
    float slope = 0.0f;
};
static inline InXform act_xform(const float* scale, const float* shift, float slope) {
    return InXform{scale, shift, slope != 0.0f ? 2 : 1, slope};
}

struct View {
    const float* p = nullptr;
    int pstride = 0;
};
struct MutView {
    float* p = nullptr;
    int pstride = 0;
};

struct ConvArgs {
// ... 49 lines not shown
    View xop, yop;
    InXform xf_x, xf_y;
    int N = 0, H = 0, W = 0;
    int Hx = 0, Wx = 0;
    int Cx = 0, Cy = 0;
    int R = 3, S = 1, pad = 1;
    float* dw = nullptr;
    int64_t tap_stride = 0;
    int sy = 0, sx = 0;
    float* slab = nullptr;
    size_t slab_floats = 0;
    double algo_flops = -1;
    bool bf16 = false;
    bool bf16x3 = false;
    int planes = 0;
};
size_t wgrad_slab_floats(const WgradArgs& a, int impl);
bool wgrad_ws_eligible(const WgradArgs& a);
void launch_wgrad_ws(rfi_ctx* ctx, const WgradArgs& a);
size_t wgrad_ws_slab_floats(const WgradArgs& a);
bool wgrad_stem_eligible(const WgradArgs& a);
void launch_wgrad_stem(rfi_ctx* ctx, const WgradArgs& a);
void launch_wgrad(rfi_ctx* ctx, const WgradArgs& a, int impl = IMPL_AUTO);

struct YRef {
    const void* p = nullptr;
    int bf16 = 0;
    int64_t ps = 0;
    YRef(const float* f) : p(f) {}
    YRef(float* f) : p(f) {}
    YRef(const float* f, int64_t pstride) : p(f), ps(pstride) {}
    YRef(const unsigned short* h, int64_t pstride) : p(h), bf16(1), ps(pstride) {}
    YRef(View v) : p(v.p), ps(v.pstride) {}
    int64_t stride(int C) const { return ps ? ps : C; }
};

size_t bn_stats_ws_floats(int C);
void launch_bn_stats(rfi_ctx* ctx, const float* y, int64_t M, int C, float* partial_ws);
void launch_bn_finalize(rfi_ctx* ctx, const float* partial_ws, int64_t M, int C, const float* gamma,
                        const float* beta, float* running_mean, float* running_var,
                        int ema_repeats, float* mean, float* invstd, float* scale, float* shift,
                        float* var_out, int records = 0,
                        hipEvent_t done = nullptr);
void launch_bn_eval_coeffs(rfi_ctx* ctx, int C, const float* gamma, const float* beta,
                           const float* running_mean, const float* running_var, float* scale,
                           float* shift);
void launch_bn_bwd_reduce(rfi_ctx* ctx, YRef da, YRef y, int64_t M, int C,
                          const float* scale, const float* shift, const float* mean,
                          const float* invstd, float* partial_ws, float* c1, float* c2,
                          float* dgamma, float* dbeta, float slope = 0.0f);
size_t bn_bwd_ws_floats(int64_t M, int C);
void launch_bn_bwd_finalize_records(rfi_ctx* ctx, const float* partial_ws, int records, int64_t M, int C, float* c1,
                                    float* c2, float* dgamma, float* dbeta);
void launch_bn_bwd_apply(rfi_ctx* ctx, YRef da_inout, YRef y, int64_t M, int C,
                         const float* scale, const float* shift, const float* mean,
                         const float* invstd, const float* gamma, const float* c1, const float* c2,
                         float* partial_ws, float* dbias, float slope = 0.0f,
                         unsigned short* planes_out = nullptr, int64_t planes_pstride = 0, int planes_P = 0,
                         hipEvent_t done = nullptr, bool finish_dbias = true, const float* head_dl = nullptr,
                         const float* head_w = nullptr);
void launch_bn_bwd_apply_finish(rfi_ctx* ctx, const float* partial_ws, int64_t M, int C, float* dbias);
struct FinishSumDesc { const double* partial; int records; int64_t stride; int count; float* out; };
int bn_bwd_apply_records(int64_t M, int C);
void launch_finish_channel_sums_batched(rfi_ctx* ctx, const FinishSumDesc* descs_dev, int n, int max_count);

void launch_bn_relu_pool(rfi_ctx* ctx, const float* y, int N, int H, int W, int C,
                         const float* scale, const float* shift, MutView skip, float* pooled, float slope = 0.0f);
void launch_pool_bwd_merge(rfi_ctx* ctx, YRef y, int N, int H, int W, int C,
                           const float* scale, const float* shift, YRef dskip, YRef dpool,
                           float* da, float slope = 0.0f, unsigned short* da16 = nullptr);
int launch_pool_bwd_merge_sums(rfi_ctx* ctx, YRef y, int N, int H, int W, int C, const float* scale,
                               const float* shift, const float* mean, const float* invstd, YRef dskip, YRef dpool,
                               float* da, float slope, float* partial_ws, unsigned short* da16 = nullptr);
void launch_head_fwd(rfi_ctx* ctx, YRef y, int64_t M, int C, const float* scale,
                     const float* shift, const float* w, const float* b, int Cout, float* logits,
                     float slope = 0.0f);
void launch_sigmoid_fwd(rfi_ctx* ctx, const float* z, int64_t n, float* x);
void launch_sigmoid_bwd(rfi_ctx* ctx, const float* x, int64_t n, float* d_inout);
void launch_loss_reduce(rfi_ctx* ctx, const float* logits, const uint8_t* labels, int64_t count,
                        double* partial_ws, double* sums4, float* loss_out);
size_t loss_ws_doubles(int64_t count);
void launch_loss_bwd(rfi_ctx* ctx, const float* logits, const uint8_t* labels, int64_t count,
                     const double* sums4, float* dlogits);
void launch_focal_reduce(rfi_ctx* ctx, const float* logits, const uint8_t* labels, int64_t count, float alpha,
                         float gamma, double* partial_ws, float* loss_out);
void launch_focal_bwd(rfi_ctx* ctx, const float* logits, const uint8_t* labels, int64_t count, float alpha,
                      float gamma, float* dlogits);
int launch_head_bwd(rfi_ctx* ctx, YRef y, int64_t M, int C, const float* scale,
                    const float* shift, const float* w, int Cout, const float* dlogits, float* da,
                    float* partial_ws, float* dw, float* db, float slope = 0.0f, const float* bn_mean = nullptr,
                    const float* bn_invstd = nullptr, float* bn_records_ws = nullptr, unsigned short* da16 = nullptr,
                    bool* skip_da = nullptr, bool finish = true);
size_t head_bwd_ws_floats(int64_t M, int C, int Cout);
void launch_channel_sum(rfi_ctx* ctx, View v, int64_t M, int C, float* partial_ws, float* out, bool finish = true);
void launch_channel_sum(rfi_ctx* ctx, YRef v, int64_t M, int C, float* partial_ws, float* out, bool finish = true);
size_t channel_sum_ws_floats(int64_t M, int C);

void launch_nchw_to_nhwc(rfi_ctx* ctx, const float* src, int N, int C, int H, int W, float* dst);
void launch_nhwc_to_nchw(rfi_ctx* ctx, const float* src, int N, int C, int H, int W, float* dst);
void launch_weight_to_dgrad(rfi_ctx* ctx, const float* wf, int taps, int Cout, int Cin, int flip,
                            float* wd);
struct RelayoutDesc {
    int64_t src_off, dst_off;
    int taps, cout, cin, flip;
    int64_t tile0 = 0;
};
int64_t relayout_assign_tiles(RelayoutDesc* descs, int n);
void launch_weight_to_dgrad_batched(rfi_ctx* ctx, const RelayoutDesc* descs_dev, int n, const float* src,
                                    float* dst, double total_bytes, int64_t total_tiles);
void launch_u8_to_f32(rfi_ctx* ctx, const uint8_t* src, int64_t n, float* dst);
void launch_relu_bwd(rfi_ctx* ctx, float* dA, const float* Y, int64_t n);
void launch_pad_channels(rfi_ctx* ctx, const float* src, int64_t M, int c, int cp, float* dst);

void launch_sumsq(rfi_ctx* ctx, const float* g, int64_t n, double* partial_ws, double* sumsq);
size_t sumsq_ws_doubles(int64_t n);
struct AdamArgs {
    float* p; float* g; float* m; float* v; int64_t n;
    float beta2, eps, wd, max_norm, grad_scale;
    float one_minus_beta1, one_minus_beta2;
    float neg_step, bc2_sqrt;
    const double* sumsq;
    float* norm_out;
};
void launch_adam(rfi_ctx* ctx, const AdamArgs& a);

void launch_preprocess(rfi_ctx* ctx, const void* patches, int dtype, int n, int ph, int pw,
                       float* minmax_ws, float* out_nhwc, const rfi_patch_src* table_dev = nullptr, int C = 0,
                       int T = 0);
void launch_patch_median(rfi_ctx* ctx, const double* v, int n, int per, bool absdev, const double* centre,
                         bool finite_only, double* out, int* cnt_out, bool f32 = false);
void launch_scale_by_median(rfi_ctx* ctx, double* v, int n, int per, const double* med, bool f32 = false);
void launch_stretch(rfi_ctx* ctx, double* v, int64_t total, int kind, bool f32 = false);
void launch_replace_inf(rfi_ctx* ctx, double* v, int n, int per, const double* mad, const int* nfinite);
void launch_mad_flags(rfi_ctx* ctx, const double* v, int n, int per, const double* med, const double* mad,
                      double sigma, uint8_t* flags, bool f32 = false);
void launch_narrow_f32(rfi_ctx* ctx, const double* src, int64_t total, float* dst);
void launch_to_abs_f64(rfi_ctx* ctx, const void* src, int dtype, int64_t total, double* dst);
void launch_synth(rfi_ctx* ctx, unsigned long long seed, int n_samples, int n_pol, int C, int T, double noise,
                  int bandpass, int order, double corr, const rfi_event* events_dev, const int* offsets_dev,
                  int out_dtype, void* planes, uint8_t* flags);
void launch_gather_labels(rfi_ctx* ctx, const uint8_t* flags, const rfi_patch_src* table_dev, int C, int T, int n,
                          int ps, uint8_t* out);
void launch_patch_any_flag(rfi_ctx* ctx, const uint8_t* flags, const rfi_patch_src* table_dev, int C, int T, int n,
                           int ps, unsigned* any_out);
void launch_confusion(rfi_ctx* ctx, const void* pred, int pred_dtype, const void* truth,
                      int truth_dtype, int64_t count, unsigned long long* counts3);
void launch_threshold(rfi_ctx* ctx, const float* logits, int64_t count, float threshold,
                      uint8_t* mask);
int64_t tiling_patches_per_plane(int C, int T, const rfi_tiling& tiling);
void check_tiling(const rfi_tiling& tiling);
void launch_stitch(rfi_ctx* ctx, const float* values, int kind, int n_planes, int C, int T, const rfi_tiling& tiling,
                   int combine, float threshold, uint8_t* flags, float* prob);
size_t flag_stats_ws_bytes();
void launch_flag_stats(rfi_ctx* ctx, const void* src, int dtype, int64_t n, const uint8_t* flags, int views,
                       bool medians, void* ws, void* mag, rfi_flag_stats* out_dev);
struct norm_chunk { const void* ptr; int64_t start; };
size_t norm_stats_ws_bytes(int pops, int64_t seg);
int norm_stats_passes(bool f32, bool quantiles);
void launch_norm_stats(rfi_ctx* ctx, const norm_chunk* chunks_dev, int n_chunks, bool f32, int64_t seg, int pops,
                       bool quantiles, const int64_t* ranks6, void* ws, rfi_norm_stats* out_dev);
void launch_norm_apply(rfi_ctx* ctx, const void* src, int dtype, bool src_nhwc, int n, int64_t px, double centre, double scale,
                       const double* params_dev, float* dst, bool dst_nhwc);
void augment_params_host(const rfi_augment_config& cfg, uint64_t call, int n, int h, int w, int32_t* gates, double* inv);
void launch_augment(rfi_ctx* ctx, const float* x, const uint8_t* y, int n, int h, int w, int c, const rfi_augment_config& cfg,
                    uint64_t call, float* x_out, uint8_t* y_out);
void launch_rfi_sim(rfi_ctx* ctx, unsigned long long seed, unsigned first_sample, int n_samples,
                    const rfi_sim_params& p, const double* power_dev, int layout, void* out, uint8_t* mask,
                    rfi_sim_event* events, double* baseline_out);

void launch_scale_inplace(rfi_ctx* ctx, float* x, int64_t n, float f);
void launch_roi_align_fwd(rfi_ctx* ctx, const float* x, int N, int H, int W, int C, const float* rois, int R, float scale,
                          int PH, int PW, int sampling_ratio, bool aligned, float* out);
void launch_roi_align_bwd(rfi_ctx* ctx, const float* dout, int N, int H, int W, int C, const float* rois, int R, float scale,
                          int PH, int PW, int sr, bool aligned, float* dx);
// ... 73 lines not shown
```

rfi_toolbox_amd/csrc/model.cpp:

```cpp
#include "model.hpp"

#include <cmath>
#include <cstdlib>
#include <random>

using namespace rfi;

namespace rfi {

void DevBuf::ensure(rfi_ctx* c, size_t floats) {
    if (floats <= n && p) return;
    if (p) c->release(p);
    ctx = c;
    p = static_cast<float*>(c->alloc(floats * sizeof(float)));
    n = floats;
}
void DevBuf::free() {
    if (p && ctx) ctx->release(p);
    p = nullptr;
    n = 0;
}

}

// ... 95 lines not shown
}

void UNetModel::prepare_shape(int n, int h, int w) {
    const int div = 1 << depth;
    RFI_REQUIRE(h % div == 0 && w % div == 0,
                "forward: H and W must be multiples of 2^depth (" + std::to_string(div) +
                    "), as the reference's pool/up-conv/cat chain requires; got " +
                    std::to_string(h) + "x" + std::to_string(w));
    if (n == pN && h == pH && w == pW && !bufs.empty()) return;
    ctx->activate();
    const int D = depth;
    if (bufs.empty()) {
        auto mk = [&](std::vector<int>& v) { v.assign(D + 1, -1); for (int l = 1; l <= D; ++l) v[l] = new_buf(); };
        mk(encY1); mk(encY2); mk(concat); mk(pool); mk(decY1); mk(decY2);
        mk(gA); mk(gB); mk(dconcat); mk(dpool); mk(gAe); mk(gBe);
        bottY1 = new_buf(); bottY2 = new_buf(); gBottA = new_buf(); gBottB = new_buf();
        logits = new_buf(); dlogits = new_buf(); probs = new_buf();
        x_stage = new_buf(); x_stage2 = new_buf(); x_pad = new_buf(); out_stage = new_buf();
        ws_red = new_buf(); ws_slab = new_buf(); lab_stage = new_buf();
    }
    size_t slab_need = 0, red_need = 0;
    auto upd_red = [&](size_t f) { if (f > red_need) red_need = f; };
    for (int l = 1; l <= D; ++l) {
        const size_t M = (size_t)n * (h >> (l - 1)) * (w >> (l - 1));
        const size_t C = (size_t)feat << (l - 1);
        for (int i : {decY1[l], decY2[l], gA[l], gB[l]}) bufs[i].ensure(ctx, M * C);
        if (!planesP && !resnet_encoder) for (int i : {gAe[l], gBe[l]}) bufs[i].ensure(ctx, M * C);
        if (!resnet_encoder) for (int i : {encY1[l], encY2[l]}) bufs[i].ensure(ctx, M * C);
        bufs[concat[l]].ensure(ctx, M * 2 * C);
        bufs[dconcat[l]].ensure(ctx, M * 2 * C);
        if (!resnet_encoder || l == D) {
            bufs[pool[l]].ensure(ctx, M / 4 * C);
            bufs[dpool[l]].ensure(ctx, M / 4 * C);
        }
    }
    {
        const size_t M = (size_t)n * (h >> D) * (w >> D);
        const size_t C = (size_t)feat << D;
        for (int i : {bottY1, bottY2, gBottA, gBottB}) bufs[i].ensure(ctx, M * C);
    }
    const size_t M1 = (size_t)n * h * w;
    bufs[logits].ensure(ctx, M1 * out_ch);
    bufs[dlogits].ensure(ctx, M1 * out_ch);
    bufs[probs].ensure(ctx, M1 * out_ch);
    bufs[x_stage].ensure(ctx, M1 * in_ch);
    bufs[x_stage2].ensure(ctx, M1 * in_ch);
    bufs[x_pad].ensure(ctx, M1 * convs[0].cin_p);
    bufs[out_stage].ensure(ctx, M1 * out_ch);
    bufs[lab_stage].ensure(ctx, (M1 + 3) / 4 + 4);
    size_t cmax = (size_t)feat << depth;
    upd_red(bn_stats_ws_floats((int)cmax));
    upd_red(bn_bwd_ws_floats(M1, (int)cmax));
    upd_red(head_bwd_ws_floats(M1, feat, out_ch) + bn_bwd_ws_floats(M1, feat));
    upd_red(channel_sum_ws_floats(M1, (int)cmax));
    upd_red(loss_ws_doubles(M1) * 2);
    upd_red(sumsq_ws_doubles(n_flat) * 2);
    bufs[ws_red].ensure(ctx, red_need + 16);
    auto conv_geom = [&](int ci, int& H, int& W) {
        H = h >> (convs[ci].level - 1);
        W = w >> (convs[ci].level - 1);
    };
    for (size_t ci = 0; ci < convs.size(); ++ci) {
        int H, W;
        conv_geom((int)ci, H, W);
        WgradArgs a;
        a.N = n; a.H = H; a.W = W; a.Hx = H; a.Wx = W;
        a.Cx = convs[ci].cin_p; a.Cy = convs[ci].cout;
        a.R = 3; a.S = 1; a.pad = 1;
        if (convs[ci].stride == 2) { a.Cx *= 4; a.R = 2; }
        if (convs[ci].R == 1) { a.R = 1; a.pad = 0; }
        a.xop.pstride = a.Cx; a.yop.pstride = a.Cy;
        a.tap_stride = (int64_t)a.Cx * a.Cy;
        a.bf16x3 = true;
        slab_need = std::max(slab_need, wgrad_slab_floats(a, IMPL_AUTO));
    }
    for (int k = 0; k < D; ++k) {
        const int l = D - k;
        WgradArgs a;
        a.N = n; a.H = h >> l; a.W = w >> l; a.Hx = a.H * 2; a.Wx = a.W * 2;
        a.Cx = ups[k].cout; a.Cy = ups[k].cin;
        a.xop.pstride = 2 * ups[k].cout; a.yop.pstride = a.Cy;
        a.R = 2; a.S = 2; a.pad = 0;
        a.tap_stride = (int64_t)a.Cx * a.Cy;
        slab_need = std::max(slab_need, wgrad_slab_floats(a, IMPL_AUTO));
    }
    bufs[ws_slab].ensure(ctx, slab_need + 16);
    if (!resnet_encoder || planesP) {
        if (dbias_pool) { ctx->release(dbias_pool); dbias_pool = nullptr; }
        if (dbias_descs) { ctx->release(dbias_descs); dbias_descs = nullptr; }
        size_t need = 0;
        std::vector<FinishSumDesc> hd;
        for (size_t ci = 0; ci < convs.size(); ++ci) {
            int H, W;
            conv_geom((int)ci, H, W);
            const int64_t M = (int64_t)n * H * W;
            convs[ci].dbias_rec_off = need;
            need += align4(channel_sum_ws_floats(M, convs[ci].cout)) + 4;
        }
        for (int k = 0; k < depth; ++k) {
            const int l = depth - k;
            ups[k].dbias_rec_off = need;
            need += align4(channel_sum_ws_floats((int64_t)n * (h >> (l - 1)) * (w >> (l - 1)), ups[k].cout)) + 4;
        }
        head_rec_off = need;
        need += align4(head_bwd_ws_floats((int64_t)n * h * w, feat, out_ch)) + 4;
        dbias_pool = static_cast<float*>(ctx->alloc(need * sizeof(float)));
// ... 266 lines not shown
    launch_conv(ctx, a);
    const int64_t M = (int64_t)s.N * s.H * s.W;
    if (train) {
        if (a.stats_records == 0) launch_bn_stats(ctx, Y, M, c.cout, ws);
        launch_bn_finalize(ctx, ws, M, c.cout, params + c.g_off, params + c.be_off, c.running_mean(), c.running_var(),
                           c.ema_repeats, c.mean(), c.invstd(), c.scale(), c.shift(), nullptr, a.stats_records);
        c.nbt += c.ema_repeats;
    } else {
        launch_bn_eval_coeffs(ctx, c.cout, params + c.g_off, params + c.be_off, c.running_mean(), c.running_var(),
                              c.scale(), c.shift());
    }
}

ConvArgs rfi_model::convt_args(const UpConv& u, View x, InXform xf, Shape s) const {
    ConvArgs a;
    a.x = x;
    a.N = s.N; a.H = s.H; a.W = s.W; a.Hin = s.H; a.Win = s.W;
    a.Cin = u.cin; a.Cout = u.cout;
    set_filters(a, params + u.w_off, u.w3);
    a.bias = params + u.b_off;
    a.Hout = 2 * s.H; a.Wout = 2 * s.W;
    a.osy = 2; a.osx = 2;
    a.R = 1; a.S = 1; a.pad = 0;
    a.zgroups = 4;
    a.xf = xf;
    return a;
}

void rfi_model::convt_backward(const UpConv& u, View dup, View x, InXform xf, Shape s, float* dx) {
    WgradArgs wa;
    wa.xop = dup;
    wa.yop = x;
    wa.xf_y = xf;
    wa.N = s.N; wa.H = s.H; wa.W = s.W; wa.Hx = 2 * s.H; wa.Wx = 2 * s.W;
    wa.Cx = u.cout; wa.Cy = u.cin;
    wa.R = 2; wa.S = 2; wa.pad = 0;
    wa.dw = grads + u.w_off;
    wa.tap_stride = (int64_t)u.cin * u.cout;
    wa.sy = 1; wa.sx = u.cin;
    set_wgrad(wa);
    wgrad_on_side(wa, nullptr);
    ConvArgs a;
    a.x = dup;
    a.N = s.N; a.H = s.H; a.W = s.W; a.Hin = 2 * s.H; a.Win = 2 * s.W;
    a.Cin = u.cout; a.Cout = u.cin;
    set_filters(a, u.wd, u.wd3);
    a.y = MutView{dx, u.cin};
    a.Hout = s.H; a.Wout = s.W;
    a.R = 2; a.S = 2; a.pad = 0;
    launch_conv(ctx, a);
}


rfi::View rfi_model::network_input(const float* x_dev, int n, int h, int w) {
    const int cp = convs[0].cin_p;
    if (cp == in_ch) return View{x_dev, in_ch};
    launch_pad_channels(ctx, x_dev, (int64_t)n * h * w, in_ch, cp, buf(x_pad));
    return View{buf(x_pad), cp};
}

void rfi_model::forward(const float* x_dev, int n, int h, int w, bool train_mode) {
    prepare(n, h, w);
    refresh_dgrad_weights();
    forward_pass(x_dev, n, h, w, train_mode);
}

void UNetModel::forward_pass(const float* x_dev, int n, int h, int w, bool train_mode) {
    if (planesP) return forward_planes(x_dev, n, h, w, train_mode);
    const int D = depth, IB = i_bott;
    auto run_conv_bn = [&](ConvBN& c, View in, InXform xf, Shape s, float* Y) {
        conv_bn(c, in, xf, s, params + c.w_off, c.w3, 3, 1, c.cin_p, Y, train_mode, 2.0 * s.N * s.H * s.W * 9.0 * c.cin * c.cout);
    };
    View cur = network_input(x_dev, n, h, w);
    if (resnet_encoder) cur = forward_resnet_encoder(cur, n, h, w, train_mode);
    else for (int l = 1; l <= D; ++l) {
        Shape s{n, h >> (l - 1), w >> (l - 1)};
        ConvBN& c1 = convs[2 * (l - 1)];
        ConvBN& c2 = convs[2 * (l - 1) + 1];
        run_conv_bn(c1, cur, InXform{}, s, buf(encY1[l]));
        if (l == 1) side_rebuild_wd();
        run_conv_bn(c2, View{buf(encY1[l]), c1.cout}, bn_xf(c1), s, buf(encY2[l]));
        launch_bn_relu_pool(ctx, buf(encY2[l]), s.N, s.H, s.W, c2.cout, c2.scale(), c2.shift(),
                            MutView{buf(concat[l]) + c2.cout, 2 * c2.cout}, buf(pool[l]), act_slope);
        cur = View{buf(pool[l]), c2.cout};
    }
    {
        Shape s{n, h >> D, w >> D};
        ConvBN& c1 = convs[IB];
        ConvBN& c2 = convs[IB + 1];
        run_conv_bn(c1, cur, InXform{}, s, buf(bottY1));
        run_conv_bn(c2, View{buf(bottY1), c1.cout}, bn_xf(c1), s, buf(bottY2));
    }
    const float* prevY = buf(bottY2);
    ConvBN* prevBN = &convs[IB + 1];
    for (int l = D; l >= 1; --l) {
        const int k = D - l;
        UpConv& u = ups[k];
        Shape sin{n, h >> l, w >> l};
        Shape s{n, h >> (l - 1), w >> (l - 1)};
        ConvArgs a = convt_args(u, View{prevY, u.cin}, bn_xf(*prevBN), sin);
        a.y = MutView{buf(concat[l]), 2 * u.cout};
        launch_conv(ctx, a);
        ConvBN& c1 = convs[IB + 2 + 2 * k];
        ConvBN& c2 = convs[IB + 2 + 2 * k + 1];
        run_conv_bn(c1, View{buf(concat[l]), 2 * u.cout}, InXform{}, s, buf(decY1[l]));
        run_conv_bn(c2, View{buf(decY1[l]), c1.cout}, bn_xf(c1), s, buf(decY2[l]));
        prevY = buf(decY2[l]);
        prevBN = &c2;
    }
    const int64_t M1 = (int64_t)n * h * w;
    launch_head_fwd(ctx, prevY, M1, feat, prevBN->scale(), prevBN->shift(), params + head_w_off,
                    params + head_b_off, out_ch, buf(logits), act_slope);
    if (head_sigmoid) launch_sigmoid_fwd(ctx, buf(logits), M1 * out_ch, buf(probs));
}

void rfi_model::loss_forward(const uint8_t* labels_dev, int n, int h, int w) {
    RFI_REQUIRE(out_ch == 1, "loss: the reference's BCE+dice step is defined for out_channels == 1");
    const int64_t cnt = (int64_t)n * h * w * out_scale * out_scale;
    if (loss_kind == 1) {
        launch_focal_reduce(ctx, buf(head_sigmoid ? probs : logits), labels_dev, cnt, focal_alpha, focal_gamma,
                            reinterpret_cast<double*>(buf(ws_red)), d_scalars);
        return;
    }
    launch_loss_reduce(ctx, buf(head_sigmoid ? probs : logits), labels_dev, cnt,
                       reinterpret_cast<double*>(buf(ws_red)), d_sums, d_scalars);
}

void rfi_model::side_begin() {
    if (!ctx->overlap) return;
    RFI_CHECK_HIP(hipEventRecord(ctx->fork_ev, ctx->main_stream));
    RFI_CHECK_HIP(hipStreamWaitEvent(ctx->side_stream, ctx->fork_ev, 0));
    ctx->stream = ctx->side_stream;
}
hipEvent_t rfi_model::next_fork_event() {
    static const bool off = getenv("RFI_NO_STOP_EVENTS") != nullptr;
    if (!ctx->overlap || off) return nullptr;
    if (ctx->fork_ring_used == ctx->fork_ring.size()) {
        hipEvent_t e;
        RFI_CHECK_HIP(hipEventCreateWithFlags(&e, hipEventDisableTiming));
        ctx->fork_ring.push_back(e);
    }
    return ctx->fork_ring[ctx->fork_ring_used++];
}
void rfi_model::side_begin_after(hipEvent_t producer_done) {
    if (!producer_done) return side_begin();
    if (!ctx->overlap) return;
    RFI_CHECK_HIP(hipStreamWaitEvent(ctx->side_stream, producer_done, 0));
    ctx->stream = ctx->side_stream;
}
void rfi_model::side_end() {
    if (!ctx->overlap) return;
    const int ring = (int)ctx->side_done.size();
    RFI_CHECK_HIP(hipEventRecord(ctx->side_done[side_seq % ring], ctx->side_stream));
    ctx->stream = ctx->main_stream;
    if (side_bound > 0 && side_seq >= side_bound)
        RFI_CHECK_HIP(hipStreamWaitEvent(ctx->main_stream, ctx->side_done[(side_seq - side_bound) % ring], 0));
    ++side_seq;
}
void rfi_model::side_join_lazy() {
    if (exchange_in_backward && ctx->exchange_active()) return side_join();
    if (!ctx->overlap || side_seq == 0) return;
    if (!lazy_ev) RFI_CHECK_HIP(hipEventCreateWithFlags(&lazy_ev, hipEventDisableTiming));
    RFI_CHECK_HIP(hipEventRecord(lazy_ev, ctx->side_stream));
    lazy_pending = true;
    side_seq = 0;
}
void rfi_model::join_pending_side() {
    if (!lazy_pending) return;
    RFI_CHECK_HIP(hipStreamWaitEvent(ctx->main_stream, lazy_ev, 0));
    lazy_pending = false;
}
// ... 9 lines not shown

static hipEvent_t bucket_event(rfi_ctx* ctx) {
    if (ctx->bucket_ev_used == ctx->bucket_ev.size()) {
        hipEvent_t e;
        RFI_CHECK_HIP(hipEventCreateWithFlags(&e, hipEventDisableTiming));
        ctx->bucket_ev.push_back(e);
    }
    return ctx->bucket_ev[ctx->bucket_ev_used++];
}
void rfi_model::bucket_ready(size_t lo, size_t hi) {
    if (!exchange_in_backward || !ctx->exchange_active() || hi <= lo) return;
    static const bool no_buckets = getenv("RFI_NO_BUCKETS") != nullptr;
    const char* mf = getenv("RFI_BUCKET_MIN_FLOATS");
    const size_t min_floats = mf ? (size_t)atoll(mf) : (size_t)1 << 20;
    if (pend_hi > pend_lo) {
        RFI_REQUIRE(hi == pend_lo || lo == pend_hi, "bucket_ready: buckets must be adjacent");
        pend_lo = std::min(pend_lo, lo);
        pend_hi = std::max(pend_hi, hi);
    } else {
        pend_lo = lo;
        pend_hi = hi;
    }
    if (no_buckets) return;
    if (pend_hi - pend_lo < min_floats && pend_lo != 0) return;
    flush_bucket();
}
void rfi_model::flush_bucket() {
    if (pend_hi <= pend_lo) return;
    const size_t lo = pend_lo, hi = pend_hi;
    pend_lo = pend_hi = 0;
    hipEvent_t em = bucket_event(ctx);
    RFI_CHECK_HIP(hipEventRecord(em, ctx->main_stream));
    RFI_CHECK_HIP(hipStreamWaitEvent(ctx->comm_stream, em, 0));
    if (ctx->overlap) {
        hipEvent_t es = bucket_event(ctx);
        RFI_CHECK_HIP(hipEventRecord(es, ctx->side_stream));
        RFI_CHECK_HIP(hipStreamWaitEvent(ctx->comm_stream, es, 0));
    }
    comm_bucket_allreduce(ctx, grads + lo, (int64_t)(hi - lo));
}
void rfi_model::exchange_join() {
    if (!ctx->exchange_active()) return;
    flush_bucket();
    hipEvent_t e = bucket_event(ctx);
    RFI_CHECK_HIP(hipEventRecord(e, ctx->comm_stream));
    RFI_CHECK_HIP(hipStreamWaitEvent(ctx->main_stream, e, 0));
    ctx->bucket_ev_used = 0;
}

namespace {

void backward_conv_bn(UNetModel* m, ConvBN& c, float* dA, const float* Y, View in, InXform in_xf,
                      Shape s, float* dx, int have_records,
                      const float* head_dl = nullptr, const float* head_w = nullptr) {
    rfi_ctx* ctx = m->ctx;
    const int64_t M = (int64_t)s.N * s.H * s.W;
    float* ws = m->buf(m->ws_red);
    if (have_records > 0)
        launch_bn_bwd_finalize_records(ctx, ws, have_records, M, c.cout, c.c1(), c.c2(), m->grads + c.g_off,
                                       m->grads + c.be_off);
    else
        launch_bn_bwd_reduce(ctx, dA, Y, M, c.cout, c.scale(), c.shift(), c.mean(), c.invstd(), ws, c.c1(),
                             c.c2(), m->grads + c.g_off, m->grads + c.be_off, m->act_slope);
    const hipEvent_t dy_done = dx ? nullptr : m->next_fork_event();
    launch_bn_bwd_apply(ctx, dA, Y, M, c.cout, c.scale(), c.shift(), c.mean(), c.invstd(),
                        m->params + c.g_off, c.c1(), c.c2(), m->dbias_deferred ? m->dbias_pool + c.dbias_rec_off : ws,
                        m->grads + c.b_off, m->act_slope, nullptr, 0, 0, dy_done, !m->dbias_deferred, head_dl, head_w);
    WgradArgs wa = m->wgrad_same(in, in_xf, dA, s, 3, 1, c.cin_p, c.cout, m->grads + c.w_off);
    wa.algo_flops = 2.0 * s.N * s.H * s.W * 9.0 * c.cin * c.cout;
    if (!dx) {
        m->wgrad_on_side(wa, dy_done);
        return;
    }
    ConvArgs a = m->conv_same(View{dA, c.cout}, InXform{}, s, 3, 1, c.cout, c.cin, c.wd, c.wd3, nullptr, dx);
    a.done = m->next_fork_event();
    launch_conv(ctx, a);
    m->wgrad_on_side(wa, a.done_used ? a.done : nullptr, !a.done_used);
}

}

void rfi_model::wgrad_on_side(const rfi::WgradArgs& wa, hipEvent_t after, bool after_everything) {
    SideScope side(this, after_everything ? nullptr : after);
    launch_wgrad(ctx, wa);
    side.end();
}

void rfi_model::backward(const float* x_dev, const uint8_t* labels_dev, int n, int h, int w) {
    join_pending_side();
    backward_pass(x_dev, labels_dev, n, h, w);
}

void UNetModel::backward_pass(const float* x_dev, const uint8_t* labels_dev, int n, int h, int w) {
    const int D = depth, IB = i_bott;
    const int64_t M1 = (int64_t)n * h * w;
    refresh_dgrad_weights();
    wait_wd();
    if (planesP) return backward_planes(x_dev, labels_dev, n, h, w);
    side_bound = resnet_encoder ? 2 : 0;
    dbias_deferred = !resnet_encoder && dbias_pool && !ctx->exchange_active();
    if (loss_kind == 1)
        launch_focal_bwd(ctx, buf(head_sigmoid ? probs : logits), labels_dev, M1, focal_alpha, focal_gamma, buf(dlogits));
    else
        launch_loss_bwd(ctx, buf(head_sigmoid ? probs : logits), labels_dev, M1, d_sums, buf(dlogits));
    if (head_sigmoid) launch_sigmoid_bwd(ctx, buf(probs), M1 * out_ch, buf(dlogits));
    int head_records = 0;
    bool head_skip = out_ch == 1;
    {
        ConvBN& last = convs[IB + 2 + 2 * (D - 1) + 1];
        const bool hdefer = dbias_deferred && head_fin_deferred;
        head_records = launch_head_bwd(ctx, buf(decY2[1]), M1, feat, last.scale(), last.shift(), params + head_w_off,
                                       out_ch, buf(dlogits), buf(gA[1]),
                                       hdefer ? dbias_pool + head_rec_off : buf(ws_red) + bn_bwd_ws_floats(M1, feat),
                                       grads + head_w_off, grads + head_b_off, act_slope, last.mean(), last.invstd(),
                                       buf(ws_red), nullptr, &head_skip, !hdefer);
    }
    for (int l = 1; l <= D; ++l) {
        const int k = D - l;
        Shape s{n, h >> (l - 1), w >> (l - 1)};
        Shape sin{n, h >> l, w >> l};
        ConvBN& c1 = convs[IB + 2 + 2 * k];
        ConvBN& c2 = convs[IB + 2 + 2 * k + 1];
        UpConv& u = ups[k];
        const bool from_head = l == 1 && head_skip;
        backward_conv_bn(this, c2, buf(gA[l]), buf(decY2[l]), View{buf(decY1[l]), c1.cout}, bn_xf(c1), s,
                         buf(gB[l]), l == 1 ? head_records : 0, from_head ? buf(dlogits) : nullptr,
                         from_head ? params + head_w_off : nullptr);
        backward_conv_bn(this, c1, buf(gB[l]), buf(decY1[l]), View{buf(concat[l]), 2 * u.cout}, InXform{}, s,
                         buf(dconcat[l]), 0);
        const float* prevY = (l == D) ? buf(bottY2) : buf(decY2[l + 1]);
        ConvBN& prevBN = (l == D) ? convs[IB + 1] : convs[IB + 2 + 2 * (k - 1) + 1];
        View dUp{buf(dconcat[l]), 2 * u.cout};
        {
            const bool defer = dbias_deferred && u.cout % 4 == 0;
            launch_channel_sum(ctx, dUp, (int64_t)s.N * s.H * s.W, u.cout, defer ? dbias_pool + u.dbias_rec_off : buf(ws_red),
                               grads + u.b_off, !defer);
        }
        convt_backward(u, dUp, View{prevY, u.cin}, bn_xf(prevBN), sin, (l == D) ? buf(gBottA) : buf(gA[l + 1]));
        bucket_ready(u.w_off, l == 1 ? n_flat : ups[k + 1].w_off);
    }
    {
        Shape s{n, h >> D, w >> D};
        ConvBN& c1 = convs[IB];
        ConvBN& c2 = convs[IB + 1];
        backward_conv_bn(this, c2, buf(gBottA), buf(bottY2), View{buf(bottY1), c1.cout}, bn_xf(c1), s, buf(gBottB), 0);
        backward_conv_bn(this, c1, buf(gBottB), buf(bottY1), View{buf(pool[D]), c1.cin}, InXform{}, s, buf(dpool[D]), 0);
        bucket_ready(c1.w_off, ups[0].w_off);
    }
    if (resnet_encoder) {
        backward_resnet_encoder(x_dev, n, h, w);
        side_join();
        return;
    }
    for (int l = D; l >= 1; --l) {
        Shape s{n, h >> (l - 1), w >> (l - 1)};
        ConvBN& c1 = convs[2 * (l - 1)];
        ConvBN& c2 = convs[2 * (l - 1) + 1];
        const std::vector<int>& gA = this->gAe;
        const std::vector<int>& gB = this->gBe;
        int have = launch_pool_bwd_merge_sums(ctx, buf(encY2[l]), s.N, s.H, s.W, c2.cout, c2.scale(), c2.shift(), c2.mean(),
                                              c2.invstd(), View{buf(dconcat[l]) + c2.cout, 2 * c2.cout}, buf(dpool[l]),
                                              buf(gA[l]), act_slope, buf(ws_red));
        if (!have)
            launch_pool_bwd_merge(ctx, buf(encY2[l]), s.N, s.H, s.W, c2.cout, c2.scale(), c2.shift(),
                                  View{buf(dconcat[l]) + c2.cout, 2 * c2.cout}, buf(dpool[l]), buf(gA[l]), act_slope);
        backward_conv_bn(this, c2, buf(gA[l]), buf(encY2[l]), View{buf(encY1[l]), c1.cout}, bn_xf(c1), s, buf(gB[l]), have);
        View in = (l == 1) ? (c1.cin_p == in_ch ? View{x_dev, in_ch} : View{buf(x_pad), c1.cin_p})
                           : View{buf(pool[l - 1]), c1.cin};
        backward_conv_bn(this, c1, buf(gB[l]), buf(encY1[l]), in, InXform{}, s,
                         (l == 1) ? nullptr : buf(dpool[l - 1]), 0);
        bucket_ready(c1.w_off, convs[l == D ? IB : 2 * l].w_off);
    }
    if (dbias_deferred) launch_finish_channel_sums_batched(ctx, static_cast<const FinishSumDesc*>(dbias_descs), dbias_n, dbias_max_c);
    side_join();
    side_bound = 2;
}

void rfi_model::apply(const rfi_hyper& hp, float grad_scale) {
    join_pending_side();
    double* ws = reinterpret_cast<double*>(buf(ws_red));
    launch_sumsq(ctx, grads, (int64_t)n_flat, ws, d_sums + 4);
    adam_step += 1;
    AdamArgs a;
    a.p = params; a.g = grads; a.m = adam_m; a.v = adam_v; a.n = (int64_t)n_flat;
    a.beta2 = (float)hp.beta2; a.eps = (float)hp.eps; a.wd = (float)hp.weight_decay;
    a.max_norm = (float)hp.max_grad_norm; a.grad_scale = grad_scale;
    a.one_minus_beta1 = (float)(1.0 - hp.beta1);
    a.one_minus_beta2 = (float)(1.0 - hp.beta2);
    a.neg_step = (float)(-(hp.lr / (1.0 - std::pow(hp.beta1, (double)adam_step))));
    a.bc2_sqrt = (float)std::sqrt(1.0 - std::pow(hp.beta2, (double)adam_step));
    a.sumsq = d_sums + 4;
    a.norm_out = d_scalars + 1;
    launch_adam(ctx, a);
    wd_dirty = true;
    x3_fresh = false;
}

void rfi_model::set_compute_dtype(int dtype) {
    arith = dtype == 1 || dtype == 4 ? Arith::BF16 : dtype == 2 || dtype == 3 ? Arith::X3 : Arith::F32;
}
void UNetModel::set_compute_dtype(int dtype) {
    rfi_model::set_compute_dtype(dtype);
    if (resnet_encoder) set_planes(dtype == 1 && feat % 16 == 0 ? 1 : 0);
    else set_planes(dtype == 1 ? 1 : (dtype == 3 ? 3 : 0));
}

void rfi_model::debug_tensor(const std::string&, const std::string&, int, bool, const float*&, size_t&) {
    throw Error("debug_tensor: this model exposes only logits / dlogits / chan (and the decoder tensors of the ResNet-encoder U-Net)");
}
void UNetModel::debug_tensor(const std::string& name, const std::string& base, int idx, bool to_host, const float*& src, size_t& n) {
    if (resnet_encoder && (base == "encY1" || base == "encY2" || base == "pool" || base == "dpool"))
        return rfi_model::debug_tensor(name, base, idx, to_host, src, n);
    RFI_REQUIRE(!(y16_flow && planesP == 1 && (base == "encY1" || base == "encY2" || base == "decY1" || base == "bottY1" ||
                                               (base == "decY2" && idx == 1))),
                "debug_tensor: this conv output is stored as bfloat16 in the bfloat16 compute mode");
    RFI_REQUIRE(!(g16_flow && planesP == 1 && (base == "gB" || base == "dpool" || base == "gBottB" || base == "gA")),
                "debug_tensor: this gradient tensor is stored as bfloat16 in the bfloat16 compute mode");
    RFI_REQUIRE(!(convt_planes && planesP == 1 && (base == "decY2" || base == "bottY2" || base == "gBottA")),
                "debug_tensor: with the transposed convs on the plane kernels this tensor is stored as bfloat16");
    const int D = depth;
    auto level = [&](const std::vector<int>& v, size_t chmul) {
        RFI_REQUIRE(idx >= 1 && idx <= D, "debug_tensor: level out of range");
        const size_t M = (size_t)pN * (pH >> (idx - 1)) * (pW >> (idx - 1));
        src = buf(v[idx]);
        n = M * ((size_t)feat << (idx - 1)) * chmul;
    };
    const size_t Mb = (size_t)pN * (pH >> D) * (pW >> D), Cb = (size_t)feat << D;
    if (base == "encY1") level(encY1, 1);
    else if (base == "encY2") level(encY2, 1);
    else if (base == "decY1") level(decY1, 1);
    else if (base == "decY2") level(decY2, 1);
    else if (base == "gA") level(!planesP && !resnet_encoder ? gAe : gA, 1);
    else if (base == "gB") level(!planesP && !resnet_encoder ? gBe : gB, 1);
    else if (base == "concat") level(concat, 2);
    else if (base == "dconcat") {
        level(dconcat, 2);
        if (convt_planes && planesP == 1 && to_host) {
            const PlaneBuf& g = pl[g16cat[idx]];
            launch_planes_to_f32(ctx, g.p, g.pstride, (int64_t)(n / ((size_t)2 * (feat << (idx - 1)))), 2 * (feat << (idx - 1)), 1,
                                 buf(dconcat[idx]), 2 * (feat << (idx - 1)));
        }
    }
    else if (base == "pool") { level(pool, 1); n /= 4; }
    else if (base == "dpool") { level(dpool, 1); n /= 4; }
// ... 26 lines not shown
```

rfi_toolbox_amd/csrc/model.hpp:

```cpp
#pragma once
#include "planes.hpp"

namespace rfi {

struct DevBuf {
    rfi_ctx* ctx = nullptr;
    float* p = nullptr;
    size_t n = 0;
    void ensure(rfi_ctx* c, size_t floats);
    void free();
};

struct PlaneBuf {
    rfi_ctx* ctx = nullptr;
    bf16_t* p = nullptr;
    size_t elems = 0;
    int64_t pstride = 0;
    int nchunks = 0;
    void ensure(rfi_ctx* c, int64_t pixels, int C, int P);
    void free();
};

struct ConvBN {
    std::string conv_name, bn_name;
// ... 117 lines not shown
    std::unordered_map<const float*, const rfi::bf16_t*> ws_by_w;
    int ws_P = 0;
    int ws_need() const { return planesP ? 0 : arith == Arith::X3 ? 3 : arith == Arith::BF16 ? 1 : 0; }
    void ws_set(rfi::ConvArgs& a) const {
        auto it = ws_by_w.find(a.w);
        const rfi::bf16_t* p = it == ws_by_w.end() || ws_P != ws_need() ? nullptr : it->second;
        a.wB3 = ws_P == 3 ? p : nullptr;
        a.wB1 = ws_P == 1 ? p : nullptr;
        if (a.wB3 && x3_skipped.count(a.w)) a.w3 = nullptr;
    }
    void set_filters(rfi::ConvArgs& a, const float* w, const float* w3) const {
        a.w = w;
        a.w3 = use_w3() ? w3 : nullptr;
        ws_set(a);
        a.bf16 = arith == Arith::BF16;
        a.bf16x3 = arith == Arith::X3;
    }
    void set_wgrad(rfi::WgradArgs& wa) const {
        wa.slab = bufs[ws_slab].p;
        wa.slab_floats = bufs[ws_slab].n;
        wa.bf16 = arith == Arith::BF16;
        wa.bf16x3 = arith == Arith::X3;
    }
    bool x3_skips_ws_layers = false;
    int ws_n_fwd = 0;
    double ws_bytes_fwd = 0;
    void refresh_ws_weights(int P, int which = 0);
    hipEvent_t wd_ready = nullptr;
    bool wd_pending = false;
    bool wd_side_todo = false;
    void side_rebuild_wd();
    bool x3_reads_wd = false;
    void wait_wd();
    void* x3_descs = nullptr;
    int x3_n = 0;
    int x3_for_ws_P = -1;
    int x3_for_shape = -1;
    std::unordered_set<const float*> x3_skipped;
    double x3_bytes = 0;
    int64_t adam_step = 0;
    bool wd_dirty = true;
    bool x3_fresh = false;
    void* relayout_descs = nullptr;
    int relayout_n = 0;
    int64_t relayout_tiles = 0;
    double relayout_bytes = 0;

    int pN = 0, pH = 0, pW = 0;
    std::vector<rfi::DevBuf> bufs;
    int logits = -1, dlogits = -1;
    int x_stage = -1, x_stage2 = -1, x_pad = -1, out_stage = -1, ws_red = -1, ws_slab = -1, lab_stage = -1;
    int gx = -1;
    bool ext_dlogits = false;
    double* d_sums = nullptr;
    float* d_scalars = nullptr;
    float last_loss = 0, last_norm = 0;

    rfi_model(int in, int out, int f, int d) : in_ch(in), out_ch(out), feat(f), depth(d) {}
    virtual ~rfi_model();
    virtual void build() = 0;
    void prepare(int n, int h, int w);
    virtual void prepare_shape(int n, int h, int w) = 0;
    void forward(const float* x_dev, int n, int h, int w, bool train_mode);
    virtual void forward_pass(const float* x_dev, int n, int h, int w, bool train_mode) = 0;
    void loss_forward(const uint8_t* labels_dev, int n, int h, int w);
    void backward(const float* x_dev, const uint8_t* labels_dev, int n, int h, int w);
    virtual void backward_pass(const float* x_dev, const uint8_t* labels_dev, int n, int h, int w) = 0;
    void apply(const rfi_hyper& hp, float grad_scale);
    virtual void algorithmic_flops(int n, int h, int w, double& fwd, double& step) const = 0;
    virtual void set_compute_dtype(int dtype);
    virtual void debug_tensor(const std::string& name, const std::string& base, int idx, bool to_host, const float*& src, size_t& n);

    size_t chan_floats = 0, wd_floats = 0;
    int add_conv(rfi::ConvBN c);
    void add_up(const std::string& name, int cin, int cout);
    void add_head(const std::string& name, int cin);
    void alloc_state();
    void reset_channel_state();
    const rfi::Entry& entry(const char* name) const;
    void init_params(uint64_t seed);
    void load_entry(const rfi::Entry& e, const void* host, size_t bytes);
    void store_entry(const rfi::Entry& e, void* host, size_t bytes);
    void store_flat(const float* flat, const rfi::Entry& e, void* host, size_t bytes);
    void load_adam(const rfi::Entry& e, const void* host_m, const void* host_v, size_t bytes);
    float* buf(int i) { return bufs[i].p; }
    int new_buf() { bufs.emplace_back(); return (int)bufs.size() - 1; }
    rfi::View network_input(const float* x_dev, int n, int h, int w);
    void refresh_dgrad_weights();
    virtual bool wd_split_ok() const { return false; }
    virtual void refresh_model_weights(int which) {}

    rfi::ConvArgs conv_same(rfi::View x, rfi::InXform xf, rfi::Shape s, int R, int pad, int cin, int cout, const float* w,
                            const float* w3, const float* bias, float* y) const;
    rfi::WgradArgs wgrad_same(rfi::View x, rfi::InXform xf_x, const float* dy, rfi::Shape s, int R, int pad, int cin, int cout,
                              float* dw) const;
    void conv_bn(rfi::ConvBN& c, rfi::View in, rfi::InXform xf, rfi::Shape s, const float* w, const float* w3, int R, int pad,
                 int cin, float* Y, bool train, double flops);
    rfi::ConvArgs convt_args(const rfi::UpConv& u, rfi::View x, rfi::InXform xf, rfi::Shape s) const;
    void convt_backward(const rfi::UpConv& u, rfi::View dup, rfi::View x, rfi::InXform xf, rfi::Shape s, float* dx);

    int side_seq = 0;
    int side_bound = 2;
    void side_begin();
    hipEvent_t next_fork_event();
    void side_begin_after(hipEvent_t producer_done);
    void side_end();
    void side_join();
    hipEvent_t lazy_ev = nullptr;
    bool lazy_pending = false;
    void side_join_lazy();
    void join_pending_side();
    void wgrad_on_side(const rfi::WgradArgs& wa, hipEvent_t after, bool after_everything = false);
    bool exchange_in_backward = false;
    void bucket_ready(size_t lo, size_t hi);
    size_t pend_lo = 0, pend_hi = 0;
    void flush_bucket();
    void exchange_join();
};

namespace rfi {
struct SideScope {
    rfi_model* m;
    bool ended = false;
    explicit SideScope(rfi_model* model, hipEvent_t after = nullptr) : m(model) { m->side_begin_after(after); }
    void end() { m->side_end(); ended = true; }
    ~SideScope() { if (!ended) m->ctx->stream = m->ctx->main_stream; }
};
}

struct UNetModel : rfi_model {
    const bool resnet_encoder;
    UNetModel(int in, int out, int f, int d, bool resnet) : rfi_model(in, out, f, d), resnet_encoder(resnet) {
        x3_skips_ws_layers = !resnet;
    }
    ~UNetModel() override;
    void build() override;
    void prepare_shape(int n, int h, int w) override;
    void forward_pass(const float* x_dev, int n, int h, int w, bool train_mode) override;
    void backward_pass(const float* x_dev, const uint8_t* labels_dev, int n, int h, int w) override;
    void algorithmic_flops(int n, int h, int w, double& fwd, double& step) const override;
// ... 140 lines not shown
```

rfi_toolbox_amd/csrc/wgrad_mfma.hip:

```cpp
#include <algorithm>

#include "planes.hpp"

namespace rfi {

void launch_wgrad_direct(rfi_ctx* ctx, const WgradArgs& a);
size_t wgrad_direct_slab_floats(const WgradArgs& a);
bool wgrad_split_eligible(const WgradArgs& a);
size_t wgrad_split_slab_floats(const WgradArgs& a);
void launch_wgrad_split(rfi_ctx* ctx, const WgradArgs& a);

namespace {

typedef float f32x4 __attribute__((ext_vector_type(4)));
typedef float f32x16 __attribute__((ext_vector_type(16)));
typedef float f32x2 __attribute__((ext_vector_type(2)));
typedef __bf16 bf16x2 __attribute__((ext_vector_type(2)));
typedef short s16x4 __attribute__((ext_vector_type(4)));
typedef unsigned u32x2 __attribute__((ext_vector_type(2)));

typedef __bf16 bf16x8 __attribute__((ext_vector_type(8)));
typedef unsigned u32x4 __attribute__((ext_vector_type(4)));
struct Split3 { bf16x8 h, m, l; };
__device__ __forceinline__ unsigned cvt_pair(float a, float b) {
// ... 352 lines not shown
}

bool wgrad_mfma_eligible(const WgradArgs& a) {
    if (a.Cx % 4 || a.Cy % 4 || a.xop.pstride % 4 || a.yop.pstride % 4) return false;
    if ((reinterpret_cast<uintptr_t>(a.xop.p) & 15) || (reinterpret_cast<uintptr_t>(a.yop.p) & 15)) return false;
    return (a.R == 3 && a.S == 1 && a.pad == 1) || (a.R == 2 && a.S == 2 && a.pad == 0);
}

Plan dispatch(rfi_ctx* ctx, const WgradArgs& a, int what, int cus) {
    if (a.R == 3) {
        const bool splits_pixels = !(a.Cy > 32 && a.Cx > 32);
        if (splits_pixels && a.H >= 16) return select<3, 1, 16, 8>(ctx, a, what, cus);
        return select<3, 1, 8, 8>(ctx, a, what, cus);
    }
    return select<2, 2, 4, 8>(ctx, a, what, cus);
}

}

size_t wgrad_slab_floats(const WgradArgs& a, int impl) {
    size_t need = wgrad_direct_slab_floats(a);
    if ((impl == IMPL_PLANES_X3 || impl == IMPL_PLANES_BF16) && a.R == 3 && a.S == 1)
        return std::max(need, pwgrad_slab_floats_f32(a));
    if (impl == IMPL_MFMA_BF16 || impl == IMPL_MFMA_BF16X3) impl = IMPL_MFMA;
    if (impl != IMPL_DIRECT && wgrad_split_eligible(a)) need = std::max(need, wgrad_split_slab_floats(a));
    if (impl != IMPL_DIRECT) need = std::max(need, wgrad_ws_slab_floats(a));
    if (impl != IMPL_DIRECT && wgrad_mfma_eligible(a)) {
        const Plan p = dispatch(nullptr, a, SEL_PLAN, 256);
        const size_t m = (size_t)p.nsplit * p.wp * p.slab_stride;
        if (m > need) need = m;
    }
    return need;
}

void launch_wgrad(rfi_ctx* ctx, const WgradArgs& a_in, int impl) {
    WgradArgs a = a_in;
    if (impl == IMPL_PLANES_X3 || impl == IMPL_PLANES_BF16) {
        RFI_REQUIRE(a.R == 3 && a.S == 1, "wgrad: the plane kernel covers 3x3 stride-1 convolutions");
        launch_pwgrad_from_f32(ctx, a, impl == IMPL_PLANES_X3 ? 3 : 1);
        return;
    }
    if (impl == IMPL_MFMA_BF16) {
        a.bf16 = true;
        impl = IMPL_MFMA;
    }
    if (impl == IMPL_MFMA_BF16X3) {
        a.bf16x3 = true;
        impl = IMPL_MFMA;
    }
    RFI_REQUIRE(a.N > 0 && a.H > 0 && a.W > 0 && a.Cx > 0 && a.Cy > 0, "wgrad: empty shape");
    RFI_REQUIRE((int64_t)a.N * a.Hx * a.Wx * a.xop.pstride < (int64_t)1 << 31 &&
                    (int64_t)a.N * a.H * a.W * a.yop.pstride < (int64_t)1 << 31,
                "wgrad: tensor too large for 32-bit element offsets");
    const bool ok = wgrad_mfma_eligible(a) || ((a.bf16 || a.bf16x3) && wgrad_split_eligible(a));
    if (impl == IMPL_MFMA) RFI_REQUIRE(ok, "wgrad: shape/alignment not eligible for the MFMA kernel");
    if (impl == IMPL_DIRECT || !ok) {
        launch_wgrad_direct(ctx, a);
        return;
    }
    if (a.bf16x3 && wgrad_stem_eligible(a)) {
        launch_wgrad_stem(ctx, a);
        return;
    }
    if ((a.bf16x3 || a.bf16) && wgrad_ws_eligible(a) && (wgrad_split_eligible(a) || (a.R == 2 && a.S == 2))) {
        launch_wgrad_ws(ctx, a);
        return;
    }
    const bool only_split = (a.R == 2 && a.S == 1) || a.R == 1;
    if (only_split) RFI_REQUIRE((a.bf16 || a.bf16x3) && wgrad_split_eligible(a),
                                "wgrad: 2x2 stride-1 and 1x1 weight gradients need the bf16 or 3 x bf16 arithmetic and 4-channel alignment");
    if ((a.bf16x3 || only_split) && wgrad_split_eligible(a)) {
        launch_wgrad_split(ctx, a);
        return;
    }
    dispatch(ctx, a, SEL_LAUNCH, 256);
}

}
```

rfi_toolbox_amd/csrc/wgrad_stem.hip:

```cpp
#include <algorithm>

#include "ws_common.hpp"

namespace rfi {
namespace {

using namespace ws;
typedef short s16x4 __attribute__((ext_vector_type(4)));
typedef __attribute__((address_space(3))) s16x4 lds_s16x4;

struct WStemDev {
    const float* x;
    const float* dy;
    int N, H, W, Cy;
    float* slab;
};

constexpr int TH = 8, TW = 16, BM = TH * TW, HH = TH + 2, HW = TW + 2, HP = HH * HW;
constexpr int ROW = 192;
constexpr int XPLANE = HP * 8;

__device__ __forceinline__ bf16x8 tr_frag(const unsigned char* p0, const unsigned char* p1) {
    const s16x4 lo = __builtin_amdgcn_ds_read_tr16_b64_v4i16((lds_s16x4*)p0);
    const s16x4 hi = __builtin_amdgcn_ds_read_tr16_b64_v4i16((lds_s16x4*)p1);
    return __builtin_bit_cast(bf16x8, __builtin_shufflevector(lo, hi, 0, 1, 2, 3, 4, 5, 6, 7));
}

template <int NT>
__global__ __launch_bounds__(256) void wgrad_stem_kernel(WStemDev d) {
    constexpr int Y_BYTES = NT * BM * ROW, X_BYTES = 3 * XPLANE;
    constexpr int RED_FLOATS = NT * 2 * 1024;
    constexpr int LDS = (Y_BYTES + X_BYTES) > RED_FLOATS * 4 ? (Y_BYTES + X_BYTES) : RED_FLOATS * 4;
    __shared__ __attribute__((aligned(16))) unsigned char smem[LDS];
    unsigned char* const sY = smem;
    unsigned char* const sX = smem + Y_BYTES;
    const int tid = threadIdx.x, lane = tid & 63, wave = tid >> 6;
    const int ll = lane & 15, q = ll >> 2, pc = ll & 3, gq = lane >> 4, kh = gq >> 1;
    const int y_lane = (gq & 1) * 32 + pc * 8;
    int x_tap[2];
#pragma unroll
    for (int cb = 0; cb < 2; ++cb) {
        const int tap = std::min(cb * 8 + (gq & 1) * 4 + pc, 8);
        x_tap[cb] = (tap / 3) * HW + tap % 3;
    }
    f32x16 acc[NT][2];
#pragma unroll
    for (int nt = 0; nt < NT; ++nt)
#pragma unroll
        for (int cb = 0; cb < 2; ++cb)
#pragma unroll
            for (int r = 0; r < 16; ++r) acc[nt][cb][r] = 0.0f;

    const int tiles_x = (d.W + TW - 1) / TW, tiles_y = (d.H + TH - 1) / TH;
    const int ntiles = d.N * tiles_y * tiles_x;
    for (int t = blockIdx.x; t < ntiles; t += gridDim.x) {
        const int ox0 = (t % tiles_x) * TW, oy0 = ((t / tiles_x) % tiles_y) * TH, n = t / (tiles_x * tiles_y);
        __syncthreads();
        for (int idx = tid; idx < BM * 8 * NT; idx += 256) {
            const int c4 = idx % (8 * NT), pix = idx / (8 * NT);
            const int y = oy0 + pix / TW, x = ox0 + pix % TW;
            f32x4 v = {0.f, 0.f, 0.f, 0.f};
            if (y < d.H && x < d.W) v = *reinterpret_cast<const f32x4*>(d.dy + ((size_t)(n * d.H + y) * d.W + x) * d.Cy + c4 * 4);
            unsigned h0, m0, l0, h1, m1, l1;
            split_pair(v.x, v.y, h0, m0, l0);
            split_pair(v.z, v.w, h1, m1, l1);
            unsigned char* dst = sY + (c4 >> 3) * (BM * ROW) + pix * ROW + (c4 & 7) * 8;
            *reinterpret_cast<u32x2*>(dst) = u32x2{h0, h1};
            *reinterpret_cast<u32x2*>(dst + 64) = u32x2{m0, m1};
            *reinterpret_cast<u32x2*>(dst + 128) = u32x2{l0, l1};
        }
        for (int idx = tid; idx < HP; idx += 256) {
            const int iy = oy0 - 1 + idx / HW, ix = ox0 - 1 + idx % HW;
            f32x4 v = {0.f, 0.f, 0.f, 0.f};
            if ((unsigned)iy < (unsigned)d.H && (unsigned)ix < (unsigned)d.W)
                v = *reinterpret_cast<const f32x4*>(d.x + ((size_t)(n * d.H + iy) * d.W + ix) * 4);
            unsigned h0, m0, l0, h1, m1, l1;
            split_pair(v.x, v.y, h0, m0, l0);
            split_pair(v.z, v.w, h1, m1, l1);
            *reinterpret_cast<u32x2*>(sX + idx * 8) = u32x2{h0, h1};
            *reinterpret_cast<u32x2*>(sX + XPLANE + idx * 8) = u32x2{m0, m1};
            *reinterpret_cast<u32x2*>(sX + 2 * XPLANE + idx * 8) = u32x2{l0, l1};
        }
        __syncthreads();
#pragma unroll
        for (int rb = 0; rb < 2; ++rb) {
            const int row = 2 * wave + rb;
            const int t0 = row * TW + 8 * kh + q, t1 = t0 + 4;
            const int h0 = row * HW + 8 * kh + q, h1 = h0 + 4;
            bf16x8 bf[2][3];
#pragma unroll
            for (int cb = 0; cb < 2; ++cb)
#pragma unroll
                for (int p = 0; p < 3; ++p)
                    bf[cb][p] = tr_frag(sX + p * XPLANE + (h0 + x_tap[cb]) * 8, sX + p * XPLANE + (h1 + x_tap[cb]) * 8);
#pragma unroll
            for (int nt = 0; nt < NT; ++nt) {
                bf16x8 af[3];
                const unsigned char* yimg = sY + nt * (BM * ROW) + y_lane;
#pragma unroll
                for (int p = 0; p < 3; ++p) af[p] = tr_frag(yimg + t0 * ROW + p * 64, yimg + t1 * ROW + p * 64);
#pragma unroll
                for (int cb = 0; cb < 2; ++cb) acc[nt][cb] = mma3(af, bf[cb], acc[nt][cb]);
            }
        }
    }
    float* s_red = reinterpret_cast<float*>(smem);
#pragma unroll
    for (int w = 1; w < 4; ++w) {
        __syncthreads();
        if (wave == w) {
#pragma unroll
            for (int nt = 0; nt < NT; ++nt)
#pragma unroll
                for (int cb = 0; cb < 2; ++cb)
#pragma unroll
                    for (int r = 0; r < 16; ++r) s_red[((nt * 2 + cb) * 16 + r) * 64 + lane] = acc[nt][cb][r];
        }
        __syncthreads();
        if (wave == 0) {
#pragma unroll
            for (int nt = 0; nt < NT; ++nt)
#pragma unroll
                for (int cb = 0; cb < 2; ++cb)
#pragma unroll
                    for (int r = 0; r < 16; ++r) acc[nt][cb][r] += s_red[((nt * 2 + cb) * 16 + r) * 64 + lane];
        }
    }
    if (wave == 0) {
        float* slab = d.slab + (size_t)blockIdx.x * 9 * d.Cy * 4;
        const int li = lane & 31, lh = lane >> 5;
#pragma unroll
        for (int cb = 0; cb < 2; ++cb) {
            const int tap = cb * 8 + (li >> 2), cx = li & 3;
            if (tap < 9) {
#pragma unroll
                for (int nt = 0; nt < NT; ++nt)
#pragma unroll
                    for (int r = 0; r < 16; ++r) {
                        const int cy = nt * 32 + (r & 3) + 8 * (r >> 2) + 4 * lh;
                        if (cy < d.Cy) slab[((size_t)tap * d.Cy + cy) * 4 + cx] = acc[nt][cb][r];
                    }
            }
        }
    }
}

}

bool wgrad_stem_eligible(const WgradArgs& a) {
    if (!(a.R == 3 && a.S == 1 && a.pad == 1 && a.Cx == 4 && a.xop.pstride == 4 && (a.Cy == 32 || a.Cy == 64) && a.yop.pstride == a.Cy)) return false;
    if (a.Hx != a.H || a.Wx != a.W || a.xf_x.scale || a.xf_y.scale) return false;
    if (a.sy != 4 || a.sx != 1 || a.tap_stride != (int64_t)4 * a.Cy) return false;
    if ((reinterpret_cast<uintptr_t>(a.xop.p) | reinterpret_cast<uintptr_t>(a.yop.p)) & 15) return false;
    return a.slab != nullptr && a.slab_floats >= (size_t)64 * 9 * a.Cy * 4;
}

void launch_wgrad_stem(rfi_ctx* ctx, const WgradArgs& a) {
    RFI_REQUIRE(wgrad_stem_eligible(a) && a.bf16x3, "wgrad_stem: shape or arithmetic not eligible");
    const int ntiles = a.N * (int)cdiv(a.H, TH) * (int)cdiv(a.W, TW);
    const int64_t stride = (int64_t)9 * a.Cy * 4;
    int GX = std::min(ntiles, a.Cy == 32 ? 1024 : 768);
    GX = (int)std::min<int64_t>(GX, (int64_t)(a.slab_floats / (size_t)stride));
    WStemDev d{a.xop.p, a.yop.p, a.N, a.H, a.W, a.Cy, a.slab};
    {
        const double flops = a.algo_flops >= 0 ? a.algo_flops : 2.0 * a.N * a.H * a.W * 9.0 * 3 * a.Cy;
        const double bytes = 4.0 * ((double)a.N * a.H * a.W * (4 + a.Cy) + 9.0 * 4 * a.Cy);
        std::string label;
        if (ctx->profiling)
            label = "wgrad_stem N" + std::to_string(a.N) + " " + std::to_string(a.H) + "x" + std::to_string(a.W) + " cx4 cy" + std::to_string(a.Cy) +
                    " split" + std::to_string(GX) + " 3xbf16";
        ProfScope ps(ctx, FAM_WGRAD_MFMA, flops, bytes, label);
        if (a.Cy == 32) hipLaunchKernelGGL(wgrad_stem_kernel<1>, dim3(GX), dim3(256), 0, ctx->stream, d);
        else hipLaunchKernelGGL(wgrad_stem_kernel<2>, dim3(GX), dim3(256), 0, ctx->stream, d);
        check_launch("wgrad_stem");
    }
    launch_reduce_slabs(ctx, a.slab, GX, stride, a.dw);
}

}
```

Baseline: 9430 patches/s.

## Fuse head conv with BCE/dice loss and read 3-channel input directly in stem

```diff
diff --git a/rfi_toolbox_amd/csrc/api.cpp b/rfi_toolbox_amd/csrc/api.cpp
--- a/rfi_toolbox_amd/csrc/api.cpp
+++ b/rfi_toolbox_amd/csrc/api.cpp
@@ -508,6 +508,11 @@
     RFI_CHECK_HIP(hipStreamSynchronize(m->ctx->stream));
     return m->ctx->pinned[0];
 }
+struct StepLabels {
+    rfi_model* m;
+    StepLabels(rfi_model* m_, const uint8_t* labels_dev) : m(m_) { m->step_labels = labels_dev; }
+    ~StepLabels() { m->step_labels = nullptr; m->head_fused = 0; }
+};
 void check_hyper(const rfi_hyper* hp) {
     RFI_REQUIRE(hp, "null hyper-parameters");
     RFI_REQUIRE(hp->lr >= 0 && hp->eps >= 0 && hp->weight_decay >= 0, "Adam: lr, eps, weight_decay must be >= 0");
@@ -559,6 +564,7 @@
         m->prepare(n, h, w);
         const float* xd = stage_input(m, x, x_mem, n, h, w, false);
         const uint8_t* yd = stage_labels(m, labels, labels_mem, n, h, w);
+        StepLabels step(m, yd);
         m->forward(xd, n, h, w, true);
         m->loss_forward(yd, n, h, w);
         m->backward(xd, yd, n, h, w);
@@ -582,6 +588,7 @@
         m->prepare(n, h, w);
         const float* xd = stage_input(m, x, x_mem, n, h, w, false);
         const uint8_t* yd = stage_labels(m, labels, labels_mem, n, h, w);
+        StepLabels step(m, yd);
         m->forward(xd, n, h, w, true);
         m->loss_forward(yd, n, h, w);
         backward_with_exchange(m, xd, yd, n, h, w);
@@ -600,6 +607,7 @@
         check_hyper(hp);
         m->ctx->activate();
         m->prepare(n, h, w);
+        StepLabels step(m, labels_dev);
         m->forward(x_dev, n, h, w, true);
         m->loss_forward(labels_dev, n, h, w);
         backward_with_exchange(m, x_dev, labels_dev, n, h, w);
diff --git a/rfi_toolbox_amd/csrc/conv_stem.hip b/rfi_toolbox_amd/csrc/conv_stem.hip
--- a/rfi_toolbox_amd/csrc/conv_stem.hip
+++ b/rfi_toolbox_amd/csrc/conv_stem.hip
@@ -9,6 +9,7 @@
 
 struct StemDev {
     const float* x;
+    int x_ps;
     int N, H, W;
     const float* w;
     const float* bias;
@@ -70,8 +71,15 @@
         for (int idx = tid; idx < HP; idx += 256) {
             const int iy = oy0 - 1 + idx / HW, ix = ox0 - 1 + idx % HW;
             f32x4 v = {0.f, 0.f, 0.f, 0.f};
-            if ((unsigned)iy < (unsigned)d.H && (unsigned)ix < (unsigned)d.W)
-                v = *reinterpret_cast<const f32x4*>(d.x + ((size_t)(n * d.H + iy) * d.W + ix) * 4);
+            if ((unsigned)iy < (unsigned)d.H && (unsigned)ix < (unsigned)d.W) {
+                const size_t pix = (size_t)(n * d.H + iy) * d.W + ix;
+                if (d.x_ps == 4) {
+                    v = *reinterpret_cast<const f32x4*>(d.x + pix * 4);
+                } else {
+                    const float* q = d.x + pix * 3;
+                    v = f32x4{q[0], q[1], q[2], 0.f};
+                }
+            }
             unsigned h0, m0, l0, h1, m1, l1;
             split_pair(v.x, v.y, h0, m0, l0);
             split_pair(v.z, v.w, h1, m1, l1);
@@ -147,10 +155,11 @@
 }
 
 bool conv_stem_eligible(const ConvArgs& a) {
-    if (!(a.R == 3 && a.S == 1 && a.pad == 1 && a.zgroups == 1 && a.Cin == 4 && a.x.pstride == 4 && (a.Cout == 32 || a.Cout == 64))) return false;
+    const bool in4 = a.Cin == 4 && a.x.pstride == 4, in3 = a.Cin == 3 && a.x.pstride == 3;
+    if (!(a.R == 3 && a.S == 1 && a.pad == 1 && a.zgroups == 1 && (in4 || in3) && (a.Cout == 32 || a.Cout == 64))) return false;
     if (a.Hin != a.H || a.Win != a.W || a.Hout != a.H || a.Wout != a.W || a.osy != 1 || a.osx != 1 || a.ooy || a.oox) return false;
     if (a.xf.scale || a.fold || a.y16) return false;
-    if ((reinterpret_cast<uintptr_t>(a.x.p) | reinterpret_cast<uintptr_t>(a.w)) & 15) return false;
+    if ((reinterpret_cast<uintptr_t>(a.x.p) & (in3 ? 3 : 15)) || (reinterpret_cast<uintptr_t>(a.w) & 15)) return false;
     return (int64_t)a.N * a.H * a.W * std::max<int64_t>(a.y.pstride, 4) * 4 < ((int64_t)1 << 40);
 }
 
@@ -161,12 +170,12 @@
     if (a.stats && GX > a.stats_max_records) GX = a.stats_max_records > 0 ? a.stats_max_records : GX;
     if (a.stats && a.stats_max_records > 0) a.stats_records = GX;
     else { a.stats = nullptr; a.stats_records = 0; }
-    StemDev d{a.x.p, a.N, a.H, a.W, a.w, a.bias, a.y.p, (int)a.y.pstride, a.Cout, a.stats};
+    StemDev d{a.x.p, (int)a.x.pstride, a.N, a.H, a.W, a.w, a.bias, a.y.p, (int)a.y.pstride, a.Cout, a.stats};
     const double flops = a.algo_flops >= 0 ? a.algo_flops : 2.0 * a.N * a.H * a.W * 9.0 * 3 * a.Cout;
-    const double bytes = 4.0 * ((double)a.N * a.H * a.W * (4 + a.Cout) + 9.0 * 4 * a.Cout);
+    const double bytes = 4.0 * ((double)a.N * a.H * a.W * (a.Cin + a.Cout) + 9.0 * 4 * a.Cout);
     std::string label;
     if (ctx->profiling)
-        label = "conv_stem N" + std::to_string(a.N) + " " + std::to_string(a.H) + "x" + std::to_string(a.W) + " 4->" + std::to_string(a.Cout) +
+        label = "conv_stem N" + std::to_string(a.N) + " " + std::to_string(a.H) + "x" + std::to_string(a.W) + " " + std::to_string(a.Cin) + "->" + std::to_string(a.Cout) +
                 " 3xbf16";
     ProfScope ps(ctx, FAM_CONV_MFMA, flops, bytes, label);
     if (a.Cout == 32) hipLaunchKernelGGL(conv_stem_kernel<1>, dim3(GX), dim3(256), 0, ctx->stream, d);
diff --git a/rfi_toolbox_amd/csrc/elem_kernels.hip b/rfi_toolbox_amd/csrc/elem_kernels.hip
--- a/rfi_toolbox_amd/csrc/elem_kernels.hip
+++ b/rfi_toolbox_amd/csrc/elem_kernels.hip
@@ -147,6 +147,25 @@
 
 __device__ __forceinline__ float act_f(float a, float slope) { return a > 0.0f ? a : (slope != 0.0f ? a * slope : 0.0f); }
 __device__ __forceinline__ float dact_f(float z, float g, float slope) { return z > 0.0f ? g : g * slope; }
+
+__device__ __forceinline__ float sigmoidf_(float x) { return 1.0f / (1.0f + expf(-x)); }
+
+struct DiceGrad {
+    float D = 1.0f, num = 0.0f, invD2 = 1.0f, invN = 1.0f;
+    __device__ __forceinline__ DiceGrad() {}
+    __device__ __forceinline__ DiceGrad(const double* __restrict__ sums4, double count) {
+        const float inter = (float)sums4[1], sp = (float)sums4[2], st = (float)sums4[3];
+        D = sp + st + 1.0f;
+        num = 2.0f * inter + 1.0f;
+        invD2 = 1.0f / (D * D);
+        invN = (float)(1.0 / count);
+    }
+    __device__ __forceinline__ float operator()(float x, float t) const {
+        const float p = sigmoidf_(x);
+        const float ddice = -(2.0f * t * D - num) * invD2;
+        return (p - t) * invN + ddice * p * (1.0f - p);
+    }
+};
 
 template <int V>
 __global__ void bn_stats_kernel(const float* __restrict__ y, int64_t M, int C, int CL,
@@ -450,7 +469,8 @@
                                     const float* __restrict__ gamma, const float* __restrict__ c1,
                                     const float* __restrict__ c2, double* __restrict__ partial, float slope,
                                     unsigned short* __restrict__ planes, int64_t pl_stride, int P,
-                                    const float* __restrict__ head_dl, const float* __restrict__ head_w) {
+                                    const float* __restrict__ head_dl, const float* __restrict__ head_w,
+                                    const uint8_t* __restrict__ head_lab, const double* __restrict__ head_sums4, double head_count) {
     __shared__ double red[V * kBlock];
     const int RL = kBlock / CL;
     const int cl = threadIdx.x % CL, rl = threadIdx.x / CL;
@@ -470,6 +490,8 @@
         float hw[V];
 #pragma unroll
         for (int v = 0; v < V; ++v) hw[v] = head_dl ? head_w[c + v] : 0.0f;
+        DiceGrad dgrad;
+        if (head_lab) dgrad = DiceGrad(head_sums4, head_count);
         constexpr int U = 4;
         for (int64_t rb = r0 + rl; rb < r1; rb += (int64_t)U * RL) {
           float yu[U][V], du[U][V];
@@ -479,7 +501,7 @@
               if (r < r1) {
                   ldy<V>(y, y16, r * yps + c, yu[k]);
                   if (head_dl) {
-                      const float d = head_dl[r];
+                      const float d = head_lab ? dgrad(head_dl[r], head_lab[r] ? 1.0f : 0.0f) : head_dl[r];
 #pragma unroll
                       for (int v = 0; v < V; ++v) du[k][v] = d * hw[v];
                   } else {
@@ -822,8 +844,6 @@
     }
 }
 
-__device__ __forceinline__ float sigmoidf_(float x) { return 1.0f / (1.0f + expf(-x)); }
-
 __global__ void loss_reduce_kernel(const float* __restrict__ logits, const uint8_t* __restrict__ labels,
                                    int64_t count, double* __restrict__ partial) {
     __shared__ double red[4][kBlock / 64];
@@ -883,19 +903,10 @@
 __global__ void loss_bwd_kernel(const float* __restrict__ logits, const uint8_t* __restrict__ labels,
                                 int64_t count, const double* __restrict__ sums4,
                                 float* __restrict__ dlogits) {
-    const float inter = (float)sums4[1], sp = (float)sums4[2], st = (float)sums4[3];
-    const float D = sp + st + 1.0f;
-    const float num = 2.0f * inter + 1.0f;
-    const float invD2 = 1.0f / (D * D);
-    const float invN = (float)(1.0 / (double)count);
+    const DiceGrad dg(sums4, (double)count);
     for (int64_t i = (int64_t)blockIdx.x * blockDim.x + threadIdx.x; i < count;
-         i += (int64_t)gridDim.x * blockDim.x) {
-        const float x = logits[i];
-        const float t = labels[i] ? 1.0f : 0.0f;
-        const float p = sigmoidf_(x);
-        const float ddice = -(2.0f * t * D - num) * invD2;
-        dlogits[i] = (p - t) * invN + ddice * p * (1.0f - p);
-    }
+         i += (int64_t)gridDim.x * blockDim.x)
+        dlogits[i] = dg(logits[i], labels[i] ? 1.0f : 0.0f);
 }
 
 __device__ __forceinline__ float focal_elem(float x, float t, float alpha, float gamma) {
@@ -1118,6 +1129,179 @@
     }
 }
 
+__global__ __launch_bounds__(256) void head_loss_fused_kernel(const float* __restrict__ y, int64_t M, int C, int CL, int64_t rows_per_block,
+                                                              const float* __restrict__ scale, const float* __restrict__ shift,
+                                                              const float* __restrict__ mean, const float* __restrict__ invstd,
+                                                              const float* __restrict__ w, const float* __restrict__ b,
+                                                              const uint8_t* __restrict__ labels, float* __restrict__ logits,
+                                                              double* __restrict__ rec, double* __restrict__ rec_b, float slope) {
+    __shared__ double red[3 * 4 * kBlock];
+    const int RL = kBlock / CL;
+    const int cl = threadIdx.x % CL, rl = threadIdx.x / CL;
+    const int c = cl * 4;
+    const bool own = c < C;
+    const int64_t r0 = (int64_t)blockIdx.x * rows_per_block;
+    int64_t r1 = r0 + rows_per_block;
+    if (r1 > M) r1 = M;
+    double acc[3][3][4], ls[7];
+#pragma unroll
+    for (int k = 0; k < 3; ++k)
+#pragma unroll
+        for (int q = 0; q < 3; ++q)
+#pragma unroll
+            for (int v = 0; v < 4; ++v) acc[k][q][v] = 0;
+#pragma unroll
+    for (int j = 0; j < 7; ++j) ls[j] = 0;
+    float sc[4] = {0, 0, 0, 0}, sh[4] = {0, 0, 0, 0}, wv[4] = {0, 0, 0, 0}, mu[4] = {0, 0, 0, 0}, is[4] = {0, 0, 0, 0};
+    if (own) { ldv<4>(scale + c, sc); ldv<4>(shift + c, sh); ldv<4>(w + c, wv); ldv<4>(mean + c, mu); ldv<4>(invstd + c, is); }
+    const float bias = b[0];
+    constexpr int U = 4;
+    for (int64_t rb = r0 + rl; rb < r1; rb += (int64_t)U * RL) {
+        float yu[U][4], tu[U];
+#pragma unroll
+        for (int k = 0; k < U; ++k) {
+            const int64_t r = rb + (int64_t)k * RL;
+#pragma unroll
+            for (int v = 0; v < 4; ++v) yu[k][v] = 0.0f;
+            tu[k] = 0.0f;
+            if (r < r1) {
+                if (own) ldv<4>(y + r * C + c, yu[k]);
+                tu[k] = labels[r] ? 1.0f : 0.0f;
+            }
+        }
+#pragma unroll
+        for (int k = 0; k < U; ++k) {
+            const int64_t r = rb + (int64_t)k * RL;
+            if (r >= r1) break;
+            float z[4], a[4];
+            float dot = 0.0f;
+#pragma unroll
+            for (int v = 0; v < 4; ++v) {
+                z[v] = yu[k][v] * sc[v] + sh[v];
+                a[v] = act_f(z[v], slope);
+                dot += a[v] * wv[v];
+            }
+            for (int off = CL >> 1; off > 0; off >>= 1) dot += __shfl_xor(dot, off, 64);
+            const float x = dot + bias;
+            const float t = tu[k];
+            const float p = sigmoidf_(x);
+            const float e2 = p * (1.0f - p);
+            const double e[3] = {(double)(p - t), (double)(t * e2), (double)e2};
+            if (cl == 0) {
+                logits[r] = x;
+                const float bce = fmaxf(x, 0.0f) - x * t + log1pf(expf(-fabsf(x)));
+                ls[0] += e[0]; ls[1] += e[1]; ls[2] += e[2];
+                ls[3] += (double)bce; ls[4] += (double)(p * t); ls[5] += (double)p; ls[6] += (double)t;
+            }
+            if (own) {
+#pragma unroll
+                for (int v = 0; v < 4; ++v) {
+                    const float gz = dact_f(z[v], wv[v], slope);
+                    const float xh = (yu[k][v] - mu[v]) * is[v];
+                    const double da = (double)a[v], dg = (double)gz, dgx = dg * (double)xh;
+#pragma unroll
+                    for (int j = 0; j < 3; ++j) {
+                        acc[j][0][v] = fma(e[j], da, acc[j][0][v]);
+                        acc[j][1][v] = fma(e[j], dg, acc[j][1][v]);
+                        acc[j][2][v] = fma(e[j], dgx, acc[j][2][v]);
+                    }
+                }
+            }
+        }
+    }
+#pragma unroll
+    for (int k = 0; k < 3; ++k) {
+        if (k) __syncthreads();
+        row_lane_reduce<4, 3>(acc[k], red, CL, RL, cl, rl);
+        if (rl == 0 && own) {
+#pragma unroll
+            for (int q = 0; q < 3; ++q)
+#pragma unroll
+                for (int v = 0; v < 4; ++v) rec[((int64_t)blockIdx.x * C + c + v) * 9 + k * 3 + q] = acc[k][q][v];
+        }
+    }
+    __syncthreads();
+    const int wave = threadIdx.x >> 6, lane = threadIdx.x & 63;
+#pragma unroll
+    for (int j = 0; j < 7; ++j) {
+        const double t = wave_sum(ls[j]);
+        if (lane == 0) red[j * (kBlock / 64) + wave] = t;
+    }
+    __syncthreads();
+    if (threadIdx.x < 8) {
+        double t = 0;
+        if (threadIdx.x < 7)
+            for (int wq = 0; wq < kBlock / 64; ++wq) t += red[threadIdx.x * (kBlock / 64) + wq];
+        rec_b[(int64_t)blockIdx.x * 8 + threadIdx.x] = t;
+    }
+}
+
+__global__ __launch_bounds__(kBlock) void head_loss_finish_kernel(const double* __restrict__ rec, const double* __restrict__ rec_b, int records,
+                                                                  int C, double count, double* __restrict__ sums4, float* __restrict__ loss_out,
+                                                                  float* __restrict__ dw, float* __restrict__ db, float* __restrict__ c1,
+                                                                  float* __restrict__ c2, float* __restrict__ dgamma, float* __restrict__ dbeta) {
+    __shared__ double red[9][kBlock / 64];
+    __shared__ double tot[4];
+    const int wave = threadIdx.x >> 6, lane = threadIdx.x & 63;
+    {
+        double s[4] = {0, 0, 0, 0};
+        for (int r = threadIdx.x; r < records; r += blockDim.x)
+            for (int k = 0; k < 4; ++k) s[k] += rec_b[(int64_t)r * 8 + 3 + k];
+#pragma unroll
+        for (int k = 0; k < 4; ++k) {
+            const double v = wave_sum(s[k]);
+            if (lane == 0) red[k][wave] = v;
+        }
+        __syncthreads();
+        if (threadIdx.x < 4) {
+            double t = 0;
+            for (int wq = 0; wq < kBlock / 64; ++wq) t += red[threadIdx.x][wq];
+            tot[threadIdx.x] = t;
+        }
+        __syncthreads();
+    }
+    const DiceGrad g(tot, count);
+    const double invN = (double)g.invN, u = -2.0 * (double)g.D * (double)g.invD2, vv = (double)g.num * (double)g.invD2;
+    const bool tail = (int)blockIdx.x == C;
+    const int nq = tail ? 3 : 9;
+    const double* src = tail ? rec_b : rec + (int64_t)blockIdx.x * 9;
+    const int64_t stride = tail ? 8 : (int64_t)C * 9;
+    double q[9] = {0, 0, 0, 0, 0, 0, 0, 0, 0};
+    for (int r = threadIdx.x; r < records; r += blockDim.x)
+#pragma unroll
+        for (int j = 0; j < 9; ++j)
+            if (j < nq) q[j] += src[(int64_t)r * stride + j];
+#pragma unroll
+    for (int j = 0; j < 9; ++j) {
+        const double v = wave_sum(q[j]);
+        if (lane == 0) red[j][wave] = v;
+    }
+    __syncthreads();
+    if (threadIdx.x != 0) return;
+    for (int j = 0; j < 9; ++j) {
+        double t = 0;
+        for (int wq = 0; wq < kBlock / 64; ++wq) t += red[j][wq];
+        q[j] = t;
+    }
+    if (tail) {
+        db[0] = (float)(invN * q[0] + u * q[1] + vv * q[2]);
+        for (int k = 0; k < 4; ++k) sums4[k] = tot[k];
+        const float bce = (float)(tot[0] / count);
+        const float inter = (float)tot[1], sp = (float)tot[2], st = (float)tot[3];
+        const float dice = 1.0f - (2.0f * inter + 1.0f) / (sp + st + 1.0f);
+        loss_out[0] = bce + dice;
+    } else {
+        const int c = blockIdx.x;
+        const double s1 = invN * q[1] + u * q[4] + vv * q[7];
+        const double s2 = invN * q[2] + u * q[5] + vv * q[8];
+        dw[c] = (float)(invN * q[0] + u * q[3] + vv * q[6]);
+        c1[c] = (float)(s1 / count);
+        c2[c] = (float)(s2 / count);
+        dgamma[c] = (float)s2;
+        dbeta[c] = (float)s1;
+    }
+}
+
 __global__ void nchw_to_nhwc_kernel(const float* __restrict__ src, int N, int C, int H, int W,
                                     float* __restrict__ dst) {
     const int64_t total = (int64_t)N * C * H * W;
@@ -1236,23 +1420,20 @@
         partial[blockIdx.x] = t;
     }
 }
-__global__ void sumsq_finish_kernel(const double* __restrict__ partial, int blocks,
-                                    double* __restrict__ out) {
-    __shared__ double red[kBlock / 64];
+__device__ __forceinline__ double sumsq_total(const double* __restrict__ partial, int blocks, double* red) {
     double s = 0;
     for (int b = threadIdx.x; b < blocks; b += blockDim.x) s += partial[b];
     s = wave_sum(s);
     if ((threadIdx.x & 63) == 0) red[threadIdx.x >> 6] = s;
     __syncthreads();
-    if (threadIdx.x == 0) {
-        double t = 0;
-        for (int k = 0; k < kBlock / 64; ++k) t += red[k];
-        out[0] = t;
-    }
-}
-
-__global__ void adam_kernel(AdamArgs a) {
-    const float norm = (float)sqrt(a.sumsq[0]) * a.grad_scale;
+    double t = 0;
+    for (int k = 0; k < kBlock / 64; ++k) t += red[k];
+    return t;
+}
+
+__global__ __launch_bounds__(kBlock) void adam_kernel(AdamArgs a) {
+    __shared__ double red[kBlock / 64];
+    const float norm = (float)sqrt(sumsq_total(a.sumsq_partial, a.sumsq_blocks, red)) * a.grad_scale;
     float coef = a.max_norm / (norm + 1e-6f);
     coef = coef > 1.0f ? 1.0f : coef;
     if (a.max_norm <= 0.0f) coef = 1.0f;
@@ -1418,8 +1599,9 @@
                          const float* invstd, const float* gamma, const float* c1, const float* c2,
                          float* partial_ws, float* dbias, float slope, unsigned short* planes_out,
                          int64_t planes_pstride, int planes_P, hipEvent_t done, bool finish_dbias, const float* head_dl,
-                         const float* head_w) {
+                         const float* head_w, const HeadLossRef* head_loss) {
     ChanGeom g = geom_rows(M, C);
+    RFI_REQUIRE(!head_loss || head_dl, "bn_bwd_apply: the fused head form needs the logits in head_dl");
     const bool fast16 = da_inout.bf16 && y.bf16 && planes_out && planes_P == 1 && !head_dl && C % 8 == 0 && da_inout.stride(C) == C &&
                         y.stride(C) % 8 == 0 && planes_pstride % 8 == 0 &&
                         !((reinterpret_cast<uintptr_t>(da_inout.p) | reinterpret_cast<uintptr_t>(y.p) | reinterpret_cast<uintptr_t>(planes_out) |
@@ -1460,7 +1642,8 @@
         auto launch = [&](auto kernel) {
             hipExtLaunchKernelGGL(kernel, dim3(g.rblocks, g.cblocks), dim3(kBlock), 0, ctx->stream, nullptr, done, 0,
                                   const_cast<void*>(da_inout.p), da_inout.bf16, y.p, y.bf16, y.stride(C), M, C, g.CL, g.rows_per_block, scale, shift, mean, invstd, gamma,
-                                  c1, c2, reinterpret_cast<double*>(partial_ws), slope, planes_out, planes_pstride, planes_P, head_dl, head_w);
+                                  c1, c2, reinterpret_cast<double*>(partial_ws), slope, planes_out, planes_pstride, planes_P, head_dl, head_w,
+                                  head_loss ? head_loss->labels : nullptr, head_loss ? head_loss->sums4 : nullptr, head_loss ? (double)head_loss->count : 1.0);
         };
         if (g.V == 4) launch(bn_bwd_apply_kernel<4>);
         else launch(bn_bwd_apply_kernel<1>);
@@ -1689,6 +1872,32 @@
 size_t head_bwd_ws_floats(int64_t M, int C, int Cout) {
     (void)M;
     return (size_t)kMaxRowBlocks * ((size_t)Cout * C + Cout) * 2;
+}
+size_t head_loss_ws_floats(int C) { return (size_t)kMaxRowBlocks * ((size_t)C * 9 + 8) * 2; }
+int launch_head_loss_fused(rfi_ctx* ctx, const float* y, int64_t M, int C, const float* scale, const float* shift,
+                           const float* mean, const float* invstd, const float* w, const float* b, const uint8_t* labels,
+                           float* logits, float* records_ws, float slope) {
+    const ChanGeom g = geom_rows(M, C);
+    const bool fits = C % 4 == 0 && g.V == 4 && g.cblocks == 1 && g.CL <= 64 &&
+                      !((reinterpret_cast<uintptr_t>(y) | reinterpret_cast<uintptr_t>(scale) | reinterpret_cast<uintptr_t>(shift) |
+                         reinterpret_cast<uintptr_t>(mean) | reinterpret_cast<uintptr_t>(invstd) | reinterpret_cast<uintptr_t>(w) |
+                         reinterpret_cast<uintptr_t>(records_ws)) & 15);
+    if (!fits) return 0;
+    RFI_REQUIRE(g.rblocks <= kMaxRowBlocks, "head_loss_fused: more row blocks than the workspace holds");
+    double* rec = reinterpret_cast<double*>(records_ws);
+    ProfScope ps(ctx, FAM_ELEMWISE, 2.0 * M * C + 27.0 * M * C, (double)M * C * 4 + (double)M * 5);
+    hipLaunchKernelGGL(head_loss_fused_kernel, dim3(g.rblocks), dim3(kBlock), 0, ctx->stream, y, M, C, g.CL, g.rows_per_block,
+                       scale, shift, mean, invstd, w, b, labels, logits, rec, rec + (size_t)g.rblocks * C * 9, slope);
+    check_launch("head_loss_fused");
+    return g.rblocks;
+}
+void launch_head_loss_finish(rfi_ctx* ctx, const float* records_ws, int records, int64_t M, int C, double* sums4,
+                             float* loss_out, float* dw, float* db, float* c1, float* c2, float* dgamma, float* dbeta) {
+    const double* rec = reinterpret_cast<const double*>(records_ws);
+    ProfScope ps(ctx, FAM_REDUCE);
+    hipLaunchKernelGGL(head_loss_finish_kernel, dim3(C + 1), dim3(kBlock), 0, ctx->stream, rec, rec + (size_t)records * C * 9,
+                       records, C, (double)M, sums4, loss_out, dw, db, c1, c2, dgamma, dbeta);
+    check_launch("head_loss_finish");
 }
 int launch_head_bwd(rfi_ctx* ctx, YRef yr, int64_t M, int C, const float* scale,
                     const float* shift, const float* w, int Cout, const float* dlogits, float* da,
@@ -1802,19 +2011,12 @@
     (void)n;
     return 1024 + 8;
 }
-void launch_sumsq(rfi_ctx* ctx, const float* g, int64_t n, double* partial_ws, double* sumsq) {
+int launch_sumsq(rfi_ctx* ctx, const float* g, int64_t n, double* partial_ws) {
     int blocks = grid_for(n / 4 + 1, 1024);
-    {
-        ProfScope ps(ctx, FAM_OPTIM, 0, (double)n * 4);
-        hipLaunchKernelGGL(sumsq_kernel, dim3(blocks), dim3(kBlock), 0, ctx->stream, g, n, partial_ws);
-        check_launch("sumsq");
-    }
-    {
-        ProfScope ps(ctx, FAM_OPTIM);
-        hipLaunchKernelGGL(sumsq_finish_kernel, dim3(1), dim3(kBlock), 0, ctx->stream, partial_ws, blocks,
-                           sumsq);
-        check_launch("sumsq_finish");
-    }
+    ProfScope ps(ctx, FAM_OPTIM, 0, (double)n * 4);
+    hipLaunchKernelGGL(sumsq_kernel, dim3(blocks), dim3(kBlock), 0, ctx->stream, g, n, partial_ws);
+    check_launch("sumsq");
+    return blocks;
 }
 void launch_adam(rfi_ctx* ctx, const AdamArgs& a) {
     ProfScope ps(ctx, FAM_OPTIM, 0, (double)a.n * 28);
diff --git a/rfi_toolbox_amd/csrc/kernels.hpp b/rfi_toolbox_amd/csrc/kernels.hpp
--- a/rfi_toolbox_amd/csrc/kernels.hpp
+++ b/rfi_toolbox_amd/csrc/kernels.hpp
@@ -125,13 +125,14 @@
 size_t bn_bwd_ws_floats(int64_t M, int C);
 void launch_bn_bwd_finalize_records(rfi_ctx* ctx, const float* partial_ws, int records, int64_t M, int C, float* c1,
                                     float* c2, float* dgamma, float* dbeta);
+struct HeadLossRef { const uint8_t* labels; const double* sums4; int64_t count; };
 void launch_bn_bwd_apply(rfi_ctx* ctx, YRef da_inout, YRef y, int64_t M, int C,
                          const float* scale, const float* shift, const float* mean,
                          const float* invstd, const float* gamma, const float* c1, const float* c2,
                          float* partial_ws, float* dbias, float slope = 0.0f,
                          unsigned short* planes_out = nullptr, int64_t planes_pstride = 0, int planes_P = 0,
                          hipEvent_t done = nullptr, bool finish_dbias = true, const float* head_dl = nullptr,
-                         const float* head_w = nullptr);
+                         const float* head_w = nullptr, const struct HeadLossRef* head_loss = nullptr);
 void launch_bn_bwd_apply_finish(rfi_ctx* ctx, const float* partial_ws, int64_t M, int C, float* dbias);
 struct FinishSumDesc { const double* partial; int records; int64_t stride; int count; float* out; };
 int bn_bwd_apply_records(int64_t M, int C);
@@ -165,6 +166,12 @@
                     const float* bn_invstd = nullptr, float* bn_records_ws = nullptr, unsigned short* da16 = nullptr,
                     bool* skip_da = nullptr, bool finish = true);
 size_t head_bwd_ws_floats(int64_t M, int C, int Cout);
+int launch_head_loss_fused(rfi_ctx* ctx, const float* y, int64_t M, int C, const float* scale, const float* shift,
+                           const float* mean, const float* invstd, const float* w, const float* b, const uint8_t* labels,
+                           float* logits, float* records_ws, float slope = 0.0f);
+void launch_head_loss_finish(rfi_ctx* ctx, const float* records_ws, int records, int64_t M, int C, double* sums4,
+                             float* loss_out, float* dw, float* db, float* c1, float* c2, float* dgamma, float* dbeta);
+size_t head_loss_ws_floats(int C);
 void launch_channel_sum(rfi_ctx* ctx, View v, int64_t M, int C, float* partial_ws, float* out, bool finish = true);
 void launch_channel_sum(rfi_ctx* ctx, YRef v, int64_t M, int C, float* partial_ws, float* out, bool finish = true);
 size_t channel_sum_ws_floats(int64_t M, int C);
@@ -185,14 +192,15 @@
 void launch_relu_bwd(rfi_ctx* ctx, float* dA, const float* Y, int64_t n);
 void launch_pad_channels(rfi_ctx* ctx, const float* src, int64_t M, int c, int cp, float* dst);
 
-void launch_sumsq(rfi_ctx* ctx, const float* g, int64_t n, double* partial_ws, double* sumsq);
+int launch_sumsq(rfi_ctx* ctx, const float* g, int64_t n, double* partial_ws);
 size_t sumsq_ws_doubles(int64_t n);
 struct AdamArgs {
     float* p; float* g; float* m; float* v; int64_t n;
     float beta2, eps, wd, max_norm, grad_scale;
     float one_minus_beta1, one_minus_beta2;
     float neg_step, bc2_sqrt;
-    const double* sumsq;
+    const double* sumsq_partial;
+    int sumsq_blocks;
     float* norm_out;
 };
 void launch_adam(rfi_ctx* ctx, const AdamArgs& a);
diff --git a/rfi_toolbox_amd/csrc/model.cpp b/rfi_toolbox_amd/csrc/model.cpp
--- a/rfi_toolbox_amd/csrc/model.cpp
+++ b/rfi_toolbox_amd/csrc/model.cpp
@@ -171,6 +171,7 @@
     upd_red(bn_stats_ws_floats((int)cmax));
     upd_red(bn_bwd_ws_floats(M1, (int)cmax));
     upd_red(head_bwd_ws_floats(M1, feat, out_ch) + bn_bwd_ws_floats(M1, feat));
+    if (out_ch == 1 && feat % 4 == 0) upd_red(head_loss_ws_floats(feat));
     upd_red(channel_sum_ws_floats(M1, (int)cmax));
     upd_red(loss_ws_doubles(M1) * 2);
     upd_red(sumsq_ws_doubles(n_flat) * 2);
@@ -543,10 +544,29 @@
 }
 
 
-rfi::View rfi_model::network_input(const float* x_dev, int n, int h, int w) {
+rfi::View rfi_model::network_input(const float* x_dev, int n, int h, int w, const ConvBN* stem) {
     const int cp = convs[0].cin_p;
     if (cp == in_ch) return View{x_dev, in_ch};
+    x_pad_valid = false;
+    if (stem) {
+        ConvArgs a = conv_same(View{x_dev, in_ch}, InXform{}, Shape{n, h, w}, 3, 1, in_ch, stem->cout, params + stem->w_off, stem->w3,
+                               nullptr, nullptr);
+        if (a.bf16x3 && conv_stem_eligible(a)) return View{x_dev, in_ch};
+    }
     launch_pad_channels(ctx, x_dev, (int64_t)n * h * w, in_ch, cp, buf(x_pad));
+    x_pad_valid = true;
+    return View{buf(x_pad), cp};
+}
+rfi::View rfi_model::network_input_bwd(const float* x_dev, int n, int h, int w, const ConvBN& stem, const float* dy) {
+    const int cp = stem.cin_p;
+    if (cp == in_ch) return View{x_dev, in_ch};
+    if (!x_pad_valid) {
+        WgradArgs wa = wgrad_same(View{x_dev, in_ch}, InXform{}, dy, Shape{n, h, w}, 3, 1, cp, stem.cout, grads + stem.w_off);
+        wa.Cx = in_ch;
+        if (wa.bf16x3 && wgrad_stem_eligible(wa)) return View{x_dev, in_ch};
+        launch_pad_channels(ctx, x_dev, (int64_t)n * h * w, in_ch, cp, buf(x_pad));
+        x_pad_valid = true;
+    }
     return View{buf(x_pad), cp};
 }
 
@@ -560,9 +580,10 @@
     if (planesP) return forward_planes(x_dev, n, h, w, train_mode);
     const int D = depth, IB = i_bott;
     auto run_conv_bn = [&](ConvBN& c, View in, InXform xf, Shape s, float* Y) {
-        conv_bn(c, in, xf, s, params + c.w_off, c.w3, 3, 1, c.cin_p, Y, train_mode, 2.0 * s.N * s.H * s.W * 9.0 * c.cin * c.cout);
+        conv_bn(c, in, xf, s, params + c.w_off, c.w3, 3, 1, in.pstride < c.cin_p ? (int)in.pstride : c.cin_p, Y, train_mode,
+                2.0 * s.N * s.H * s.W * 9.0 * c.cin * c.cout);
     };
-    View cur = network_input(x_dev, n, h, w);
+    View cur = network_input(x_dev, n, h, w, resnet_encoder ? nullptr : &convs[0]);
     if (resnet_encoder) cur = forward_resnet_encoder(cur, n, h, w, train_mode);
     else for (int l = 1; l <= D; ++l) {
         Shape s{n, h >> (l - 1), w >> (l - 1)};
@@ -600,6 +621,19 @@
         prevBN = &c2;
     }
     const int64_t M1 = (int64_t)n * h * w;
+    head_fused = 0;
+    if (train_mode && step_labels && loss_kind == 0 && out_ch == 1 && out_scale == 1 && !head_sigmoid && feat % 4 == 0 &&
+        !resnet_encoder) {
+        head_fused_records = launch_head_loss_fused(ctx, prevY, M1, feat, prevBN->scale(), prevBN->shift(), prevBN->mean(),
+                                                    prevBN->invstd(), params + head_w_off, params + head_b_off, step_labels,
+                                                    buf(logits), buf(ws_red), act_slope);
+        if (head_fused_records) {
+            head_fused = 1;
+            head_fused_labels = step_labels;
+            head_fused_conv = (int)(prevBN - convs.data());
+            return;
+        }
+    }
     launch_head_fwd(ctx, prevY, M1, feat, prevBN->scale(), prevBN->shift(), params + head_w_off,
                     params + head_b_off, out_ch, buf(logits), act_slope);
     if (head_sigmoid) launch_sigmoid_fwd(ctx, buf(logits), M1 * out_ch, buf(probs));
@@ -608,6 +642,14 @@
 void rfi_model::loss_forward(const uint8_t* labels_dev, int n, int h, int w) {
     RFI_REQUIRE(out_ch == 1, "loss: the reference's BCE+dice step is defined for out_channels == 1");
     const int64_t cnt = (int64_t)n * h * w * out_scale * out_scale;
+    if (head_fused == 1 && labels_dev == head_fused_labels) {
+        ConvBN& last = convs[head_fused_conv];
+        launch_head_loss_finish(ctx, buf(ws_red), head_fused_records, cnt, feat, d_sums, d_scalars, grads + head_w_off,
+                                grads + head_b_off, last.c1(), last.c2(), grads + last.g_off, grads + last.be_off);
+        head_fused = 2;
+        return;
+    }
+    head_fused = 0;
     if (loss_kind == 1) {
         launch_focal_reduce(ctx, buf(head_sigmoid ? probs : logits), labels_dev, cnt, focal_alpha, focal_gamma,
                             reinterpret_cast<double*>(buf(ws_red)), d_scalars);
@@ -723,11 +765,13 @@
 
 void backward_conv_bn(UNetModel* m, ConvBN& c, float* dA, const float* Y, View in, InXform in_xf,
                       Shape s, float* dx, int have_records,
-                      const float* head_dl = nullptr, const float* head_w = nullptr) {
+                      const float* head_dl = nullptr, const float* head_w = nullptr, const HeadLossRef* head_loss = nullptr) {
     rfi_ctx* ctx = m->ctx;
     const int64_t M = (int64_t)s.N * s.H * s.W;
     float* ws = m->buf(m->ws_red);
-    if (have_records > 0)
+    if (head_loss)
+        ;
+    else if (have_records > 0)
         launch_bn_bwd_finalize_records(ctx, ws, have_records, M, c.cout, c.c1(), c.c2(), m->grads + c.g_off,
                                        m->grads + c.be_off);
     else
@@ -736,8 +780,9 @@
     const hipEvent_t dy_done = dx ? nullptr : m->next_fork_event();
     launch_bn_bwd_apply(ctx, dA, Y, M, c.cout, c.scale(), c.shift(), c.mean(), c.invstd(),
                         m->params + c.g_off, c.c1(), c.c2(), m->dbias_deferred ? m->dbias_pool + c.dbias_rec_off : ws,
-                        m->grads + c.b_off, m->act_slope, nullptr, 0, 0, dy_done, !m->dbias_deferred, head_dl, head_w);
+                        m->grads + c.b_off, m->act_slope, nullptr, 0, 0, dy_done, !m->dbias_deferred, head_dl, head_w, head_loss);
     WgradArgs wa = m->wgrad_same(in, in_xf, dA, s, 3, 1, c.cin_p, c.cout, m->grads + c.w_off);
+    if (in.pstride < c.cin_p) wa.Cx = (int)in.pstride;
     wa.algo_flops = 2.0 * s.N * s.H * s.W * 9.0 * c.cin * c.cout;
     if (!dx) {
         m->wgrad_on_side(wa, dy_done);
@@ -770,14 +815,18 @@
     if (planesP) return backward_planes(x_dev, labels_dev, n, h, w);
     side_bound = resnet_encoder ? 2 : 0;
     dbias_deferred = !resnet_encoder && dbias_pool && !ctx->exchange_active();
-    if (loss_kind == 1)
-        launch_focal_bwd(ctx, buf(head_sigmoid ? probs : logits), labels_dev, M1, focal_alpha, focal_gamma, buf(dlogits));
-    else
-        launch_loss_bwd(ctx, buf(head_sigmoid ? probs : logits), labels_dev, M1, d_sums, buf(dlogits));
-    if (head_sigmoid) launch_sigmoid_bwd(ctx, buf(probs), M1 * out_ch, buf(dlogits));
+    const bool fused = head_fused == 2 && labels_dev && labels_dev == head_fused_labels && !ext_dlogits &&
+                       head_fused_conv == IB + 2 + 2 * (D - 1) + 1;
+    head_fused = 0;
+    const HeadLossRef head_loss{labels_dev, d_sums, M1};
     int head_records = 0;
     bool head_skip = out_ch == 1;
-    {
+    if (!fused) {
+        if (loss_kind == 1)
+            launch_focal_bwd(ctx, buf(head_sigmoid ? probs : logits), labels_dev, M1, focal_alpha, focal_gamma, buf(dlogits));
+        else
+            launch_loss_bwd(ctx, buf(head_sigmoid ? probs : logits), labels_dev, M1, d_sums, buf(dlogits));
+        if (head_sigmoid) launch_sigmoid_bwd(ctx, buf(probs), M1 * out_ch, buf(dlogits));
         ConvBN& last = convs[IB + 2 + 2 * (D - 1) + 1];
         const bool hdefer = dbias_deferred && head_fin_deferred;
         head_records = launch_head_bwd(ctx, buf(decY2[1]), M1, feat, last.scale(), last.shift(), params + head_w_off,
@@ -794,9 +843,10 @@
         ConvBN& c2 = convs[IB + 2 + 2 * k + 1];
         UpConv& u = ups[k];
         const bool from_head = l == 1 && head_skip;
+        const bool from_loss = l == 1 && fused;
         backward_conv_bn(this, c2, buf(gA[l]), buf(decY2[l]), View{buf(decY1[l]), c1.cout}, bn_xf(c1), s,
-                         buf(gB[l]), l == 1 ? head_records : 0, from_head ? buf(dlogits) : nullptr,
-                         from_head ? params + head_w_off : nullptr);
+                         buf(gB[l]), l == 1 ? head_records : 0, from_head ? buf(from_loss ? logits : dlogits) : nullptr,
+                         from_head ? params + head_w_off : nullptr, from_loss ? &head_loss : nullptr);
         backward_conv_bn(this, c1, buf(gB[l]), buf(decY1[l]), View{buf(concat[l]), 2 * u.cout}, InXform{}, s,
                          buf(dconcat[l]), 0);
         const float* prevY = (l == D) ? buf(bottY2) : buf(decY2[l + 1]);
@@ -836,13 +886,14 @@
             launch_pool_bwd_merge(ctx, buf(encY2[l]), s.N, s.H, s.W, c2.cout, c2.scale(), c2.shift(),
                                   View{buf(dconcat[l]) + c2.cout, 2 * c2.cout}, buf(dpool[l]), buf(gA[l]), act_slope);
         backward_conv_bn(this, c2, buf(gA[l]), buf(encY2[l]), View{buf(encY1[l]), c1.cout}, bn_xf(c1), s, buf(gB[l]), have);
-        View in = (l == 1) ? (c1.cin_p == in_ch ? View{x_dev, in_ch} : View{buf(x_pad), c1.cin_p})
-                           : View{buf(pool[l - 1]), c1.cin};
+        View in = (l == 1) ? network_input_bwd(x_dev, n, h, w, c1, buf(gB[l])) : View{buf(pool[l - 1]), c1.cin};
         backward_conv_bn(this, c1, buf(gB[l]), buf(encY1[l]), in, InXform{}, s,
                          (l == 1) ? nullptr : buf(dpool[l - 1]), 0);
         bucket_ready(c1.w_off, convs[l == D ? IB : 2 * l].w_off);
     }
-    if (dbias_deferred) launch_finish_channel_sums_batched(ctx, static_cast<const FinishSumDesc*>(dbias_descs), dbias_n, dbias_max_c);
+    if (dbias_deferred)
+        launch_finish_channel_sums_batched(ctx, static_cast<const FinishSumDesc*>(dbias_descs),
+                                           dbias_n - (fused && head_fin_deferred ? 2 : 0), dbias_max_c);
     side_join();
     side_bound = 2;
 }
@@ -850,7 +901,7 @@
 void rfi_model::apply(const rfi_hyper& hp, float grad_scale) {
     join_pending_side();
     double* ws = reinterpret_cast<double*>(buf(ws_red));
-    launch_sumsq(ctx, grads, (int64_t)n_flat, ws, d_sums + 4);
+    const int sumsq_blocks = launch_sumsq(ctx, grads, (int64_t)n_flat, ws);
     adam_step += 1;
     AdamArgs a;
     a.p = params; a.g = grads; a.m = adam_m; a.v = adam_v; a.n = (int64_t)n_flat;
@@ -860,7 +911,7 @@
     a.one_minus_beta2 = (float)(1.0 - hp.beta2);
     a.neg_step = (float)(-(hp.lr / (1.0 - std::pow(hp.beta1, (double)adam_step))));
     a.bc2_sqrt = (float)std::sqrt(1.0 - std::pow(hp.beta2, (double)adam_step));
-    a.sumsq = d_sums + 4;
+    a.sumsq_partial = ws; a.sumsq_blocks = sumsq_blocks;
     a.norm_out = d_scalars + 1;
     launch_adam(ctx, a);
     wd_dirty = true;
diff --git a/rfi_toolbox_amd/csrc/model.hpp b/rfi_toolbox_amd/csrc/model.hpp
--- a/rfi_toolbox_amd/csrc/model.hpp
+++ b/rfi_toolbox_amd/csrc/model.hpp
@@ -193,6 +193,9 @@
     int x_stage = -1, x_stage2 = -1, x_pad = -1, out_stage = -1, ws_red = -1, ws_slab = -1, lab_stage = -1;
     int gx = -1;
     bool ext_dlogits = false;
+    const uint8_t* step_labels = nullptr;
+    int head_fused = 0, head_fused_records = 0, head_fused_conv = -1;
+    const uint8_t* head_fused_labels = nullptr;
     double* d_sums = nullptr;
     float* d_scalars = nullptr;
     float last_loss = 0, last_norm = 0;
@@ -226,7 +229,9 @@
     void load_adam(const rfi::Entry& e, const void* host_m, const void* host_v, size_t bytes);
     float* buf(int i) { return bufs[i].p; }
     int new_buf() { bufs.emplace_back(); return (int)bufs.size() - 1; }
-    rfi::View network_input(const float* x_dev, int n, int h, int w);
+    rfi::View network_input(const float* x_dev, int n, int h, int w, const rfi::ConvBN* stem = nullptr);
+    rfi::View network_input_bwd(const float* x_dev, int n, int h, int w, const rfi::ConvBN& stem, const float* dy);
+    bool x_pad_valid = false;
     void refresh_dgrad_weights();
     virtual bool wd_split_ok() const { return false; }
     virtual void refresh_model_weights(int which) {}
diff --git a/rfi_toolbox_amd/csrc/wgrad_mfma.hip b/rfi_toolbox_amd/csrc/wgrad_mfma.hip
--- a/rfi_toolbox_amd/csrc/wgrad_mfma.hip
+++ b/rfi_toolbox_amd/csrc/wgrad_mfma.hip
@@ -428,6 +428,10 @@
     RFI_REQUIRE((int64_t)a.N * a.Hx * a.Wx * a.xop.pstride < (int64_t)1 << 31 &&
                     (int64_t)a.N * a.H * a.W * a.yop.pstride < (int64_t)1 << 31,
                 "wgrad: tensor too large for 32-bit element offsets");
+    if (impl != IMPL_DIRECT && a.bf16x3 && a.Cx == 3 && wgrad_stem_eligible(a)) {
+        launch_wgrad_stem(ctx, a);
+        return;
+    }
     const bool ok = wgrad_mfma_eligible(a) || ((a.bf16 || a.bf16x3) && wgrad_split_eligible(a));
     if (impl == IMPL_MFMA) RFI_REQUIRE(ok, "wgrad: shape/alignment not eligible for the MFMA kernel");
     if (impl == IMPL_DIRECT || !ok) {
diff --git a/rfi_toolbox_amd/csrc/wgrad_stem.hip b/rfi_toolbox_amd/csrc/wgrad_stem.hip
--- a/rfi_toolbox_amd/csrc/wgrad_stem.hip
+++ b/rfi_toolbox_amd/csrc/wgrad_stem.hip
@@ -11,6 +11,7 @@
 
 struct WStemDev {
     const float* x;
+    int x_ps;
     const float* dy;
     int N, H, W, Cy;
     float* slab;
@@ -72,8 +73,15 @@
         for (int idx = tid; idx < HP; idx += 256) {
             const int iy = oy0 - 1 + idx / HW, ix = ox0 - 1 + idx % HW;
             f32x4 v = {0.f, 0.f, 0.f, 0.f};
-            if ((unsigned)iy < (unsigned)d.H && (unsigned)ix < (unsigned)d.W)
-                v = *reinterpret_cast<const f32x4*>(d.x + ((size_t)(n * d.H + iy) * d.W + ix) * 4);
+            if ((unsigned)iy < (unsigned)d.H && (unsigned)ix < (unsigned)d.W) {
+                const size_t pix = (size_t)(n * d.H + iy) * d.W + ix;
+                if (d.x_ps == 4) {
+                    v = *reinterpret_cast<const f32x4*>(d.x + pix * 4);
+                } else {
+                    const float* q = d.x + pix * 3;
+                    v = f32x4{q[0], q[1], q[2], 0.f};
+                }
+            }
             unsigned h0, m0, l0, h1, m1, l1;
             split_pair(v.x, v.y, h0, m0, l0);
             split_pair(v.z, v.w, h1, m1, l1);
@@ -148,10 +156,11 @@
 }
 
 bool wgrad_stem_eligible(const WgradArgs& a) {
-    if (!(a.R == 3 && a.S == 1 && a.pad == 1 && a.Cx == 4 && a.xop.pstride == 4 && (a.Cy == 32 || a.Cy == 64) && a.yop.pstride == a.Cy)) return false;
+    const bool in4 = a.Cx == 4 && a.xop.pstride == 4, in3 = a.Cx == 3 && a.xop.pstride == 3;
+    if (!(a.R == 3 && a.S == 1 && a.pad == 1 && (in4 || in3) && (a.Cy == 32 || a.Cy == 64) && a.yop.pstride == a.Cy)) return false;
     if (a.Hx != a.H || a.Wx != a.W || a.xf_x.scale || a.xf_y.scale) return false;
     if (a.sy != 4 || a.sx != 1 || a.tap_stride != (int64_t)4 * a.Cy) return false;
-    if ((reinterpret_cast<uintptr_t>(a.xop.p) | reinterpret_cast<uintptr_t>(a.yop.p)) & 15) return false;
+    if ((reinterpret_cast<uintptr_t>(a.xop.p) & (in3 ? 3 : 15)) || (reinterpret_cast<uintptr_t>(a.yop.p) & 15)) return false;
     return a.slab != nullptr && a.slab_floats >= (size_t)64 * 9 * a.Cy * 4;
 }
 
@@ -161,13 +170,13 @@
     const int64_t stride = (int64_t)9 * a.Cy * 4;
     int GX = std::min(ntiles, a.Cy == 32 ? 1024 : 768);
     GX = (int)std::min<int64_t>(GX, (int64_t)(a.slab_floats / (size_t)stride));
-    WStemDev d{a.xop.p, a.yop.p, a.N, a.H, a.W, a.Cy, a.slab};
+    WStemDev d{a.xop.p, (int)a.xop.pstride, a.yop.p, a.N, a.H, a.W, a.Cy, a.slab};
     {
         const double flops = a.algo_flops >= 0 ? a.algo_flops : 2.0 * a.N * a.H * a.W * 9.0 * 3 * a.Cy;
-        const double bytes = 4.0 * ((double)a.N * a.H * a.W * (4 + a.Cy) + 9.0 * 4 * a.Cy);
+        const double bytes = 4.0 * ((double)a.N * a.H * a.W * (a.Cx + a.Cy) + 9.0 * 4 * a.Cy);
         std::string label;
         if (ctx->profiling)
-            label = "wgrad_stem N" + std::to_string(a.N) + " " + std::to_string(a.H) + "x" + std::to_string(a.W) + " cx4 cy" + std::to_string(a.Cy) +
+            label = "wgrad_stem N" + std::to_string(a.N) + " " + std::to_string(a.H) + "x" + std::to_string(a.W) + " cx" + std::to_string(a.Cx) + " cy" + std::to_string(a.Cy) +
                     " split" + std::to_string(GX) + " 3xbf16";
         ProfScope ps(ctx, FAM_WGRAD_MFMA, flops, bytes, label);
         if (a.Cy == 32) hipLaunchKernelGGL(wgrad_stem_kernel<1>, dim3(GX), dim3(256), 0, ctx->stream, d);
```

Result: no change. 9396 patches/s (-0.4%).
